# brson/synth2

Hardware: AMD Instinct MI355X
Metric: voice-samples/sec (mono) at 64k voices per GPU, 48 kHz, 1024-frame buffers (higher is better)
Workload: dtype f32

## Files before the change

### synth2_amd/csrc/s2r_aux.hip

```cpp
#include "s2r_kern_common.h"

namespace {

__global__ void __launch_bounds__(256) s2r_table_kernel(const S2rTabBuild b) {
    __shared__ uint64_t sT[S2R_EXP2F_N];
    if (threadIdx.x < S2R_EXP2F_N) sT[threadIdx.x] = c_exp2f_table[threadIdx.x];
    __syncthreads();
    const uint32_t i = blockIdx.x * blockDim.x + threadIdx.x;
    if (i >= b.n_entries) return;
    const S2rEnv &e = b.mod;
    float mod;
    bool dead = false;
    if (i < b.n_ad) {
        const float t = (float)i;
        const EnvRun s = env_stage_at(e, __builtin_inff(), __builtin_inff(), t);
        mod = env_value(s, t);
    } else if (i < b.n_ad + b.n_rel) {
        const float t = (float)(b.rc_t0 + (i - b.n_ad));
        mod = e.slope_rel * (t - e.sus_off) + e.S;
    } else if (i < b.n_ad + 2u * b.n_rel) {
        const float d = (float)(i - b.n_ad - b.n_rel);
        mod = e.slope_rel * d + e.S;
    } else if (i < b.n_ad + 2u * b.n_rel + 16u) {
        mod = 0.0f * 1.0f + e.S;
    } else {
        mod = 0.0f;
        dead = i >= b.n_ad + 2u * b.n_rel + 32u;
    }
    const float f_lpf = s2r_pow2_sleef_core(mod * b.amt_lpf) * b.lpf_freq;
    float c0, c1, c2 = 0.0f;
    if (b.lpf_kind == S2R_FILT_ONEPOLE) {
        const float num = (-2.0f * 3.14159274101257324f) * f_lpf;
        const float arg = b.fast_div_sr ? s2r_div_const_nocheck(num, b.sr, b.rcp_sr) : (num / b.sr);
        c0 = s2r_expf(arg, sT);
        c1 = 1.0f - c0;
        if (dead) { c0 = 1.0f; c1 = 0.0f; }
    } else {
        const FiltCoef fc = dsp_filter_coef(b.lpf_kind, b.lpf_damping, b.sr, f_lpf);
        c0 = fc.alpha; c1 = fc.beta; c2 = fc.gamma;
        if (dead) c0 = 1.0f;
    }
    b.base[i] = c0;
    b.base[(size_t)b.plane + i] = c1;
    if (b.lpf_kind != S2R_FILT_ONEPOLE) b.base[2u * (size_t)b.plane + i] = c2;
    if (b.fm_plane) b.base[(size_t)b.fm_plane * b.plane + i] = dead ? 1.0f : s2r_pow2_sleef_core(mod * b.amt_osc);
}

__global__ void __launch_bounds__(256) s2r_noise_table_kernel(float *t) {
    const uint32_t x = blockIdx.x * blockDim.x + threadIdx.x;
    const float f = (float)((x * 0x79b9u) & 0xffffu) * 0x1p-16f;
    const float q = __builtin_fmaf(f, 0x1.0001p-16f, f);
    t[x] = __builtin_fmaf(q, 2.0f, -1.0f);
}

__device__ __forceinline__ void mix_body(const S2rMixParams &m, uint32_t block, float *s_run) {
    const bool ov = m.ov_render_counter != nullptr;
    if (ov) {
        if (threadIdx.x == 0 && !ov_wait(m.ov_render_counter, m.ov_render_target)) ov_raise(m.ov_fail, 2u);
        __syncthreads();
    }
    mix_block(m, block, s_run, ov, m.done.flag != nullptr);
    signal_done(m.done, (m.frames + 15u) / 16u);
}

__global__ void __launch_bounds__(256) s2r_mix_kernel(const S2rMixParams m) {
    extern __shared__ float s_run[];
    tl_mark(m.timeline, m.tl_slot, 0);
    mix_body(m, blockIdx.x, s_run);
    tl_mark(m.timeline, m.tl_slot, 1);
}

__global__ void s2r_sum_rows_kernel(const float *rows, uint32_t n_rows, uint32_t frames, uint32_t stride, int stereo, float *out, const S2rDone done) {
    const uint32_t f = blockIdx.x * blockDim.x + threadIdx.x;
    if (f < frames) {
        float total = 0.0f;
        for (uint32_t r = 0; r < n_rows; ++r) total += rows[(size_t)r * stride + f];
        if (stereo) { out_store(done, out + 2u * f, total); out_store(done, out + 2u * f + 1u, total); }
        else out_store(done, out + f, total);
    }
    signal_done(done, gridDim.x);
}

constexpr int kDecimTaps = 63;
__global__ void s2r_decimate4_kernel(const float *x, const float *h, uint32_t n_out, float *out) {
    const uint32_t n = blockIdx.x * blockDim.x + threadIdx.x;
    if (n >= n_out) return;
    float acc = 0.0f;
    for (int k = 0; k < kDecimTaps; ++k) acc = acc + h[k] * x[4u * n + (uint32_t)k];
    out[n] = acc;
}
__global__ void s2r_decimate4_history_kernel(float *x, uint32_t n_out) {
    const uint32_t i = threadIdx.x;
    float v = 0.0f;
    if (i < kDecimTaps - 1) v = x[4u * n_out + i];
    __syncthreads();
    if (i < kDecimTaps - 1) x[i] = v;
}

__device__ __forceinline__ void heads_body(int32_t *heads, const S2rTimedEvent *tev, S2rTimedEvent *tev_copy, uint32_t n, uint32_t i, bool ov) {
    if (i >= n) return;
    const S2rTimedEvent e = tev[i];
    if (ov) {
        static_assert(sizeof(S2rTimedEvent) == 32, "two 16-byte stores");
        float *dst = reinterpret_cast<float *>(tev_copy + i);
        ov_store4(dst, (f4){s2r_u2f(e.voice), s2r_u2f(e.frame), s2r_u2f(e.flags), e.pitch});
        ov_store4(dst + 4, (f4){s2r_u2f(e.seed), s2r_u2f((uint32_t)e.next), s2r_u2f(e.program), 0.0f});
        if (e.flags & S2R_TEV_FIRST) ov_store(heads + e.voice, (int32_t)i);
    } else {
        tev_copy[i] = e;
        if (e.flags & S2R_TEV_FIRST) heads[e.voice] = (int32_t)i;
    }
}

__global__ void s2r_tev_heads_kernel(int32_t *heads, const S2rTimedEvent *tev, S2rTimedEvent *tev_copy, uint32_t n, uint32_t *ov_heads_counter) {
    heads_body(heads, tev, tev_copy, n, blockIdx.x * blockDim.x + threadIdx.x, ov_heads_counter != nullptr);
    if (ov_heads_counter != nullptr) ov_signal(ov_heads_counter);
}

__global__ void __launch_bounds__(256) s2r_mix_and_heads_kernel(const S2rMixParams m, uint32_t mix_blocks, int32_t *heads,
                                                                const S2rTimedEvent *tev, S2rTimedEvent *tev_copy, uint32_t n) {
    extern __shared__ float s_run[];
    tl_mark(m.timeline, m.tl_slot, 0);
    if (blockIdx.x < mix_blocks) mix_body(m, blockIdx.x, s_run);
    else {
        heads_body(heads, tev, tev_copy, n, (blockIdx.x - mix_blocks) * blockDim.x + threadIdx.x, m.ov_heads_counter != nullptr);
        if (m.ov_heads_counter != nullptr) ov_signal(m.ov_heads_counter);
    }
    tl_mark(m.timeline, m.tl_slot, 1);
}

__global__ void s2r_events_kernel(const S2rVoiceArrays v, const S2rVoiceEvent *ev, uint32_t n) {
    const uint32_t i = blockIdx.x * blockDim.x + threadIdx.x;
    if (i >= n) return;
    const S2rVoiceEvent e = ev[i];
    const uint32_t vi = e.voice;
    if (e.flags & S2R_EV_RESTART) {
        v.pitch[vi] = e.pitch;
        v.offset[vi] = 0u;
        v.release[vi] = 0u;
        v.flags[vi] = S2R_VF_STARTED | ((e.flags & S2R_EV_RELEASE) ? S2R_VF_RELEASED : 0u);
        v.phase[vi] = 0.0f;
        v.lpf_last[vi] = 0.0f;
        v.fx1[vi] = 0.0f; v.fx2[vi] = 0.0f; v.fy1[vi] = 0.0f; v.fy2[vi] = 0.0f;
        v.seed[vi] = e.seed;
        v.program[vi] = e.flags >> S2R_EV_PROGRAM_SHIFT;
        v.osc_z[vi] = s2r_u2f(S2R_OSC_Z_NONE);
    } else if (e.flags & S2R_EV_RELEASE) {
        const uint32_t fl = v.flags[vi];
        if ((fl & S2R_VF_STARTED) && !(fl & S2R_VF_RELEASED)) {
            v.release[vi] = v.offset[vi];
            v.flags[vi] = fl | S2R_VF_RELEASED;
        }
    }
}
}

hipError_t s2r_launch_onepole_resident_osc0(const S2rRenderArgs &a, const S2rResident &rs, uint32_t block_voices, hipStream_t stream);
hipError_t s2r_launch_onepole_resident_osc1(const S2rRenderArgs &a, const S2rResident &rs, uint32_t block_voices, hipStream_t stream);
hipError_t s2r_launch_onepole_resident_osc2(const S2rRenderArgs &a, const S2rResident &rs, uint32_t block_voices, hipStream_t stream);
hipError_t s2r_launch_onepole_resident_osc3(const S2rRenderArgs &a, const S2rResident &rs, uint32_t block_voices, hipStream_t stream);
hipError_t s2r_launch_onepole_pool_osc0(const S2rRenderArgs &a, const S2rPool &pl, uint32_t block_voices, hipStream_t stream);
hipError_t s2r_launch_onepole_pool_osc1(const S2rRenderArgs &a, const S2rPool &pl, uint32_t block_voices, hipStream_t stream);
hipError_t s2r_launch_onepole_pool_osc2(const S2rRenderArgs &a, const S2rPool &pl, uint32_t block_voices, hipStream_t stream);
hipError_t s2r_launch_onepole_pool_osc3(const S2rRenderArgs &a, const S2rPool &pl, uint32_t block_voices, hipStream_t stream);
hipError_t s2r_launch_onepole_osc0(const S2rRenderArgs &a, uint32_t block_voices, hipStream_t stream);
hipError_t s2r_launch_onepole_osc1(const S2rRenderArgs &a, uint32_t block_voices, hipStream_t stream);
hipError_t s2r_launch_onepole_osc2(const S2rRenderArgs &a, uint32_t block_voices, hipStream_t stream);
hipError_t s2r_launch_onepole_osc3(const S2rRenderArgs &a, uint32_t block_voices, hipStream_t stream);
hipError_t s2r_launch_general_pool_osc0(const S2rRenderArgs &a, const S2rPool &pl, uint32_t block_voices, hipStream_t stream);
hipError_t s2r_launch_general_pool_osc1(const S2rRenderArgs &a, const S2rPool &pl, uint32_t block_voices, hipStream_t stream);
hipError_t s2r_launch_general_pool_osc2(const S2rRenderArgs &a, const S2rPool &pl, uint32_t block_voices, hipStream_t stream);
hipError_t s2r_launch_general_pool_osc3(const S2rRenderArgs &a, const S2rPool &pl, uint32_t block_voices, hipStream_t stream);
hipError_t s2r_launch_general_pool_osc15(const S2rRenderArgs &a, const S2rPool &pl, uint32_t block_voices, hipStream_t stream);
hipError_t s2r_launch_general_osc0(const S2rRenderArgs &a, uint32_t block_voices, hipStream_t stream);
hipError_t s2r_launch_general_osc1(const S2rRenderArgs &a, uint32_t block_voices, hipStream_t stream);
hipError_t s2r_launch_general_osc2(const S2rRenderArgs &a, uint32_t block_voices, hipStream_t stream);
hipError_t s2r_launch_general_osc3(const S2rRenderArgs &a, uint32_t block_voices, hipStream_t stream);
hipError_t s2r_launch_general_osc15(const S2rRenderArgs &a, uint32_t block_voices, hipStream_t stream);

hipError_t s2r_launch_tables(const S2rTabBuild &b, hipStream_t stream) {
    if (b.n_entries == 0) return hipErrorInvalidValue;
    hipLaunchKernelGGL(s2r_table_kernel, dim3((b.n_entries + 255u) / 256u), dim3(256), 0, stream, b);
    return hipGetLastError();
}

hipError_t s2r_launch_noise_table(float *table_65536, hipStream_t stream) {
    hipLaunchKernelGGL(s2r_noise_table_kernel, dim3(65536 / 256), dim3(256), 0, stream, table_65536);
    return hipGetLastError();
}

hipError_t s2r_launch_render(const S2rRenderArgs &a, uint32_t block_voices, hipStream_t stream) {
    const S2rRenderParams &p = a.p;
    if (p.n_voices == 0 || p.frames == 0) return hipSuccess;
    if (block_voices < 64 || block_voices > 1024 || (block_voices & 63u)) return hipErrorInvalidValue;
    if (p.bank_size > 1 || p.osc_kind > S2R_OSC_SINE) return s2r_launch_general_osc15(a, block_voices, stream);
    const bool general = p.lpf_kind != S2R_FILT_ONEPOLE;
    switch (p.osc_kind) {
    case S2R_OSC_SQUARE: return general ? s2r_launch_general_osc0(a, block_voices, stream) : s2r_launch_onepole_osc0(a, block_voices, stream);
    case S2R_OSC_SAW: return general ? s2r_launch_general_osc1(a, block_voices, stream) : s2r_launch_onepole_osc1(a, block_voices, stream);
    case S2R_OSC_TRIANGLE: return general ? s2r_launch_general_osc2(a, block_voices, stream) : s2r_launch_onepole_osc2(a, block_voices, stream);
    case S2R_OSC_SINE: return general ? s2r_launch_general_osc3(a, block_voices, stream) : s2r_launch_onepole_osc3(a, block_voices, stream);
    default: return hipErrorInvalidValue;
    }
}

hipError_t s2r_launch_resident(const S2rRenderArgs &a, const S2rResident &rs, uint32_t block_voices, hipStream_t stream) {
    const S2rRenderParams &p = a.p;
    if (p.n_voices == 0 || p.frames == 0 || p.bank_size > 1 || p.lpf_kind != S2R_FILT_ONEPOLE) return hipErrorInvalidValue;
    switch (p.osc_kind) {
    case S2R_OSC_SQUARE: return s2r_launch_onepole_resident_osc0(a, rs, block_voices, stream);
    case S2R_OSC_SAW: return s2r_launch_onepole_resident_osc1(a, rs, block_voices, stream);
    case S2R_OSC_TRIANGLE: return s2r_launch_onepole_resident_osc2(a, rs, block_voices, stream);
    case S2R_OSC_SINE: return s2r_launch_onepole_resident_osc3(a, rs, block_voices, stream);
    default: return hipErrorInvalidValue;
    }
}

hipError_t s2r_launch_pool(const S2rRenderArgs &a, const S2rPool &pl, uint32_t block_voices, hipStream_t stream) {
    const S2rRenderParams &p = a.p;
    if (p.n_voices == 0 || p.frames == 0) return hipErrorInvalidValue;
    if (p.bank_size > 1 || p.osc_kind > S2R_OSC_SINE) return s2r_launch_general_pool_osc15(a, pl, block_voices, stream);
    const bool general = p.lpf_kind != S2R_FILT_ONEPOLE;
    switch (p.osc_kind) {
    case S2R_OSC_SQUARE: return general ? s2r_launch_general_pool_osc0(a, pl, block_voices, stream) : s2r_launch_onepole_pool_osc0(a, pl, block_voices, stream);
    case S2R_OSC_SAW: return general ? s2r_launch_general_pool_osc1(a, pl, block_voices, stream) : s2r_launch_onepole_pool_osc1(a, pl, block_voices, stream);
    case S2R_OSC_TRIANGLE: return general ? s2r_launch_general_pool_osc2(a, pl, block_voices, stream) : s2r_launch_onepole_pool_osc2(a, pl, block_voices, stream);
    case S2R_OSC_SINE: return general ? s2r_launch_general_pool_osc3(a, pl, block_voices, stream) : s2r_launch_onepole_pool_osc3(a, pl, block_voices, stream);
    default: return hipErrorInvalidValue;
    }
}

hipError_t s2r_launch_mix(const S2rMixParams &m, hipStream_t stream) {
    if (m.frames == 0) return hipSuccess;
    const uint32_t runs_per_group = (m.blocks_per_group + kMixRun - 1) / kMixRun;
    const size_t lds = (size_t)runs_per_group * m.n_groups * 16u * sizeof(float);
    if (lds > 64u * 1024u) return hipErrorInvalidValue;
    hipLaunchKernelGGL(s2r_mix_kernel, dim3((m.frames + 15) / 16), dim3(256), lds, stream, m);
    return hipGetLastError();
}

hipError_t s2r_launch_mix_and_heads(const S2rMixParams &m, int32_t *heads, const S2rTimedEvent *tev, S2rTimedEvent *tev_copy, uint32_t n,
                                    hipStream_t stream) {
    if (m.frames == 0) return s2r_launch_tev_heads(heads, tev, tev_copy, n, stream, m.ov_heads_counter);
    if (n == 0) return s2r_launch_mix(m, stream);
    const uint32_t runs_per_group = (m.blocks_per_group + kMixRun - 1) / kMixRun;
    const size_t lds = (size_t)runs_per_group * m.n_groups * 16u * sizeof(float);
    if (lds > 64u * 1024u) return hipErrorInvalidValue;
    const uint32_t mix_blocks = (m.frames + 15) / 16;
    hipLaunchKernelGGL(s2r_mix_and_heads_kernel, dim3(mix_blocks + (n + 255) / 256), dim3(256), lds, stream, m, mix_blocks, heads, tev, tev_copy, n);
    return hipGetLastError();
}

hipError_t s2r_launch_events(const S2rVoiceArrays &v, const S2rVoiceEvent *dev_events, uint32_t n, hipStream_t stream) {
    if (n == 0) return hipSuccess;
    hipLaunchKernelGGL(s2r_events_kernel, dim3((n + 255) / 256), dim3(256), 0, stream, v, dev_events, n);
    return hipGetLastError();
}

hipError_t s2r_launch_tev_heads(int32_t *heads, const S2rTimedEvent *tev, S2rTimedEvent *tev_copy, uint32_t n, hipStream_t stream,
                                uint32_t *ov_heads_counter) {
    if (n == 0) return hipSuccess;
    hipLaunchKernelGGL(s2r_tev_heads_kernel, dim3((n + 255) / 256), dim3(256), 0, stream, heads, tev, tev_copy, n, ov_heads_counter);
    return hipGetLastError();
}

hipError_t s2r_launch_decimate4(float *x_with_history, const float *taps, uint32_t n_out, float *out, hipStream_t stream) {
    if (n_out == 0) return hipSuccess;
    hipLaunchKernelGGL(s2r_decimate4_kernel, dim3((n_out + 255) / 256), dim3(256), 0, stream, x_with_history, taps, n_out, out);
// ... 12 lines not shown
```

### synth2_amd/csrc/s2r_device.h

```cpp
#pragma once
#include <hip/hip_runtime_api.h>
#include <stdint.h>
#include "s2r.h"

#define S2R_VF_STARTED 1u
#define S2R_VF_RELEASED 2u

struct S2rEnv {
    float A;
    float D;
    float S;
    float R;
    float sus_off;
    float slope_att;
    float slope_dec;
    float slope_rel;
};

struct S2rVoiceArrays {
    float *pitch;
    uint32_t *offset;
    uint32_t *release;
    uint32_t *flags;
    float *phase;
// ... 8 lines not shown

struct S2rBankEntry {
    int32_t osc_kind;
    float osc_gain, noise_level, lpf_freq, amt_osc, amt_lpf;
    int32_t lpf_kind;
    float lpf_shape;
    S2rEnv amp, mod;
    uint32_t tab_valid;
    uint32_t tab_off, tab_plane;
    int32_t tab_ad, tab_rc;
    uint32_t tab_rc_t0;
    int32_t tab_ru, tab_sus, tab_end, tab_dead;
};

struct S2rTimedEvent;

struct S2rDone {
    uint32_t *flag;
    uint32_t value;
    uint32_t *counter;
};

struct S2rTabRef {
    const float *base;
    uint32_t plane;
    int32_t ad;
    int32_t rc;
    uint32_t rc_t0;
    int32_t ru;
    int32_t sus;
    int32_t end;
    int32_t dead;
    uint32_t fm_plane;
};
#define S2R_TAB_PAD 16u
#define S2R_TAB_MAX_ENTRIES (1u << 22)

struct S2rMixTail {
    uint32_t n_mixers;
    uint32_t n_blocks, blocks_per_group, n_groups;
    int32_t root_add, stereo;
    float *out;
    S2rDone done;
    uint32_t *rows_done;
    uint32_t rows_target;
    int32_t xmode;
    uint32_t n_rows, row_stride;
    const float *rows;
    float *final_out;
    S2rDone final_done;
    int32_t final_stereo;
    unsigned long long *granules;
    uint32_t granule_tag;
};

struct S2rRenderParams {
    int32_t osc_kind;
    float osc_gain;
    float noise_level;
    float lpf_freq;
    float amt_osc;
    float amt_lpf;
    int32_t lpf_kind;
    float lpf_damping;
    S2rEnv amp;
    S2rEnv mod;
    float sr;
    float rcp_sr;
    int32_t fast_div_sr;
    int32_t no_flat_shortcut;
    uint32_t frames;
    uint32_t n_voices;
    uint32_t frames_stride;
    uint32_t super_frames;
    S2rVoiceArrays v;
    float *block_partials;
    float *direct_out;
    int32_t direct_stereo;
    S2rDone done;
    float *per_voice;
    const float *sin_table;
    const float *noise_tab;
    S2rTabRef tab;
    const S2rTimedEvent *tev;
    int32_t *voice_ev_head;
    unsigned long long *stamps;
    unsigned long long *timeline;
    uint32_t tl_slot;
    const S2rBankEntry *bank;
    uint32_t bank_size;
    const uint32_t *ov_heads_counter;
    uint32_t ov_heads_target;
    uint32_t *ov_render_counter;
    uint32_t *ov_fail;
    const S2rTimedEvent *tev_src;
    S2rTimedEvent *tev_copy;
    const uint32_t *slices;
    uint32_t *arrive;
    uint32_t arrive_target;
    S2rMixTail mt;
};

struct S2rVoiceEvent {
    uint32_t voice;
    uint32_t flags;
    float pitch;
    uint32_t seed;
};
#define S2R_EV_RESTART 1u
#define S2R_EV_RELEASE 2u
#define S2R_EV_PROGRAM_SHIFT 16

struct S2rTimedEvent {
    uint32_t voice;
    uint32_t frame;
    uint32_t flags;
    float pitch;
    uint32_t seed;
    int32_t next;
    uint32_t program;
    uint32_t _pad;
};
#define S2R_TEV_FIRST 0x100u

#define S2R_ARG_MAX_EVENTS 288u
struct S2rRenderArgs {
    S2rRenderParams p;
    uint32_t n_events;
    uint32_t _pad;
    uint32_t ev[3 * S2R_ARG_MAX_EVENTS];
};
static_assert(sizeof(S2rRenderArgs) <= 4096, "kernel arguments are limited to 4 KiB");

#define S2R_RES_CMD_WORDS 32u
#define S2R_RES_MAX_EVENTS 9u
#define S2R_RES_FLAG_EXIT 1u
#define S2R_RES_GRANULE_FRAMES 64u
struct S2rResident {
    const uint32_t *cmd;
    uint32_t *exited;
    uint32_t launch_id;
    uint32_t first_seq;
    uint32_t idle_ticks;
    uint32_t max_polls;
    uint32_t *done_flag, *done_counter;
    unsigned long long *granules;
};

#define S2R_POOL_CMD_SLOTS 4u
#define S2R_POOL_CMD_WORDS 16u
#define S2R_POOL_FLAG_EXIT 1u
#define S2R_POOL_FLAG_TWO_STREAMS 2u
struct S2rPool {
    const uint32_t *cmd;
    const uint32_t *slices;
    uint32_t slices_stride;
    const S2rTimedEvent *tev_src[4];
    S2rTimedEvent *tev_copy[2];
    int32_t *heads[2];
    float *partials[2];
    uint32_t *arrive;
    const uint32_t *ov_heads;
    uint32_t *ov_render;
    float *out[3];
    uint32_t *done_flag, *done_counter;
    uint32_t *decided;
    uint32_t *exited;
    uint32_t *fail;
    uint32_t launch_id, first_seq, idle_ticks, max_polls;
    S2rMixTail mt;
    float *rows[2], *rows_mine[2];
    float *final_out[3];
    uint32_t *final_flag, *final_counter;
    unsigned long long *granules;
};

struct S2rTabBuild {
    S2rEnv mod;
    float lpf_freq, amt_lpf, amt_osc, sr, rcp_sr;
    int32_t fast_div_sr;
    int32_t lpf_kind;
    float lpf_damping;
    float *base;
    uint32_t plane, n_ad, n_rel, n_entries;
    uint32_t rc_t0;
    uint32_t fm_plane;
};

struct S2rOverlapWords { uint32_t render_done[2], heads_done[2]; };

struct S2rMixParams {
    const float *block_partials;
    uint32_t n_blocks;
    uint32_t blocks_per_group;
    uint32_t n_groups;
    uint32_t frames;
    uint32_t frames_stride;
    int32_t root_add;
    int32_t stereo;
    float *out;
    S2rDone done;
    const uint32_t *ov_render_counter;
    uint32_t ov_render_target;
    uint32_t *ov_heads_counter;
    uint32_t *ov_fail;
    unsigned long long *timeline;
    uint32_t tl_slot;
    unsigned long long *granules;
    uint32_t granule_tag;
};

hipError_t s2r_launch_tables(const S2rTabBuild &b, hipStream_t stream);
hipError_t s2r_launch_noise_table(float *table_65536, hipStream_t stream);
hipError_t s2r_launch_resident(const S2rRenderArgs &a, const S2rResident &rs, uint32_t block_voices, hipStream_t stream);
hipError_t s2r_launch_render(const S2rRenderArgs &a, uint32_t block_voices, hipStream_t stream);
hipError_t s2r_launch_pool(const S2rRenderArgs &a, const S2rPool &pl, uint32_t block_voices, hipStream_t stream);
hipError_t s2r_launch_mix(const S2rMixParams &p, hipStream_t stream);
hipError_t s2r_launch_events(const S2rVoiceArrays &v, const S2rVoiceEvent *dev_events, uint32_t n, hipStream_t stream);
hipError_t s2r_launch_mix_and_heads(const S2rMixParams &m, int32_t *heads, const S2rTimedEvent *tev, S2rTimedEvent *tev_copy, uint32_t n,
                                    hipStream_t stream);
hipError_t s2r_launch_tev_heads(int32_t *heads, const S2rTimedEvent *tev, S2rTimedEvent *tev_copy, uint32_t n, hipStream_t stream,
                                uint32_t *ov_heads_counter = nullptr);
hipError_t s2r_launch_decimate4(float *x_with_history, const float *taps, uint32_t n_out, float *out, hipStream_t stream);
hipError_t s2r_launch_sum_rows(const float *rows, uint32_t n_rows, uint32_t frames, uint32_t stride, int stereo, float *out, hipStream_t stream,
                               const S2rDone *done);
```

### synth2_amd/csrc/s2r_host.cpp

```cpp
#include <hip/hip_runtime.h>
#include <cmath>
#include <cstdarg>
#include <cstdio>
#include <cstdlib>
#include <cstring>
#include <ctime>
#include <atomic>
#include <memory>
#include <new>
#include <string>
#include <vector>

#include "s2r.h"
#include "s2r_device.h"
#include "s2r_math.h"
#include "s2r_patch.h"
#include "s2r_voices.h"

namespace {

constexpr int kEventSlots = 4;
constexpr size_t kVoiceWords = S2R_VOICE_WORDS;

constexpr uint32_t kSinTableCrc = 0x55293b66u;
// ... 92 lines not shown
    int device = 0;
    uint32_t shard_begin = 0, shard_voices = 0, padded_voices = 0, block_voices = 256, n_blocks = 0, mix_groups = 1;
    uint32_t interleave = 0, shard_index = 0, shard_count = 1;
    FastDiv div_interleave, div_count, div_per_kid;
    std::vector<s2r_patch> bank;
    uint32_t program = 0;
    S2rBankEntry *bank_dev = nullptr;
    bool bank_dirty = true; uint32_t bank_rate = 0;
    std::shared_ptr<S2rVoicePool> pool;
    s2r_synth *parent = nullptr;
    std::vector<s2r_synth *> kids;
    float *rows_dev[2] = {nullptr, nullptr};
    std::vector<float *> kid_stage;
    std::vector<hipEvent_t> kid_done[2];
    uint32_t rows_slot = 0;
    std::vector<uint32_t> seed_override;
    std::vector<S2rVoiceEvent> pending;
    std::vector<int32_t> pending_slot;
    EventSlot slots[kEventSlots];
    int next_slot = 0;
    std::vector<S2rTimedEvent> tpending;
    std::vector<int32_t> tlast;
    std::vector<int32_t> tfirst;
    uint32_t fill_time = 0;
    uint32_t tev_capacity = 0;
    int32_t *voice_ev_head = nullptr;
    S2rTimedEvent *tev_copy = nullptr;
    hipStream_t stream = nullptr;
    S2rVoiceArrays v{};
    void *voice_mem = nullptr;
    float *block_partials = nullptr;
    float *out_dev = nullptr;
    float *out_host = nullptr;
    float *out_host_dev = nullptr;
    uint32_t *done_host = nullptr, *done_dev = nullptr, *done_counter = nullptr;
    uint32_t done_seq = 0;
    uint32_t ring_seq[2] = {0, 0};
    float *ring_host[2] = {nullptr, nullptr}, *ring_dev[2] = {nullptr, nullptr};
    hipEvent_t ring_done[2] = {nullptr, nullptr};
    size_t ring_frames[2] = {0, 0};
    uint32_t ring_head = 0, ring_count = 0;
    struct DeferredMix { bool active = false; bool overlap = false; S2rMixParams m{}; int ring_slot = -1; } dmix;
    hipStream_t stream_b = nullptr;
    bool ov_enabled = false;
    bool ov_registered = false;
    bool ov_busy = false;
    float *partials2[2] = {nullptr, nullptr};
    int32_t *heads2[2] = {nullptr, nullptr};
    S2rTimedEvent *tevcopy2[2] = {nullptr, nullptr};
    S2rOverlapWords *ov_words = nullptr;
    uint32_t ov_render_target[2] = {0, 0}, ov_heads_target[2] = {0, 0};
    uint32_t ov_fill = 0;
    int fused_mode = 1;
    uint32_t *fz_arrive = nullptr;
    uint32_t fz_target[2] = {0, 0};
    FastDiv div_block;
    std::vector<S2rTimedEvent> tsorted;
    std::vector<uint32_t> tperm, tbounds;
    uint32_t *rows_done = nullptr;
    uint32_t rows_target[2] = {0, 0};
    bool xg_on = false;
    uint32_t xg_rank = 0, xg_n = 0, xg_target[2] = {0, 0};
    float *xg_rows = nullptr;
    uint32_t *xg_done = nullptr;
    void *xg_block = nullptr; bool xg_owner = false;
    bool force_stage = false, force_peer = false;
    bool resident = false, pool_running = false;
    uint32_t pool_seq = 0, pool_launch_id = 0, pool_rate = 0, pool_fills = 0;
    uint32_t *pool_cmd = nullptr, *pool_cmd_dev = nullptr; bool pool_cmd_vram = false;
    uint32_t *pool_slices = nullptr, *pool_slices_dev = nullptr;
    uint32_t *pool_host = nullptr, *pool_host_dev = nullptr;
    uint32_t *pool_decided = nullptr;
    bool pool_gran_pending = false;
    EventSlot *pool_gran_slot = nullptr;
    volatile uint32_t *pool_staged = nullptr; uint32_t pool_staged_seq = 0;
    uint32_t pool_idle_ticks = 200000u;
    int n_cu = 0;
    float *os_buf = nullptr, *os_taps = nullptr;
    float *sin_dev = nullptr;
    float *noise_dev = nullptr;
    float *per_voice_dev = nullptr; size_t per_voice_cap = 0;
    float *tab_dev = nullptr; size_t tab_cap = 0;
    S2rTabRef tab{};
    bool tab_dirty = true; uint32_t tab_rate = 0;
    float *bank_tab_dev = nullptr; size_t bank_tab_cap = 0;
    unsigned long long *stamps_dev = nullptr;
    unsigned long long *timeline_dev = nullptr; uint32_t timeline_n = 0, timeline_cap = 0;
    bool use_tab = true, use_arg_events = true;
    bool low_latency = false, res_running = false, res_stereo = false;
    uint32_t res_rate = 0, res_seq = 0, res_launch_id = 0;
    uint32_t *res_host = nullptr, *res_dev = nullptr;
    unsigned long long *res_gran = nullptr, *res_gran_dev = nullptr;
    uint32_t *res_cmd = nullptr;
    uint32_t *res_cmd_dev = nullptr;
    bool res_cmd_vram = false;
    float pitch_table[256];
    hipEvent_t t0 = nullptr, t1 = nullptr;
    bool timing = false, timed = false, no_flat_shortcut = false;
    uint64_t double_release = 0;
    s2r_voice_log_fn voice_log = nullptr;
    void *voice_log_user = nullptr;
    bool broken = false;
    std::string err = "";
};


namespace {

int set_err(s2r_synth *s, int code, const char *fmt, ...) {
    if (s) {
        char buf[512];
        va_list ap; va_start(ap, fmt); vsnprintf(buf, sizeof buf, fmt, ap); va_end(ap);
        s->err = buf;
    }
    return code;
}

#define S2R_QUIESCE(s) do { const int rc_q_ = quiesce(s); if (rc_q_ != S2R_OK) return rc_q_; } while (0)
int resident_stop(s2r_synth *s);
int pool_stop(s2r_synth *s);
int quiesce(s2r_synth *s) { int rc = resident_stop(s); return rc != S2R_OK ? rc : pool_stop(s); }

#define S2R_HIP(s, call)                                                                              \
    do {                                                                                              \
        hipError_t e_ = (call);                                                                       \
        if (e_ != hipSuccess) return set_err((s), S2R_ERR_HIP, "%s failed: %s", #call, hipGetErrorString(e_)); \
    } while (0)

inline int64_t to_local(const s2r_synth *s, uint32_t pool_index) {
    if (s->interleave == 0) {
        if (pool_index < s->shard_begin || pool_index >= s->shard_begin + s->shard_voices) return -1;
        return (int64_t)(pool_index - s->shard_begin);
    }
    const uint32_t run = s->div_interleave.div(pool_index), within = pool_index - run * s->interleave;
    const uint32_t lrun = s->div_count.div(run);
    if (run - lrun * s->shard_count != s->shard_index) return -1;
    return (int64_t)(lrun * s->interleave + within);
}
inline uint32_t to_pool(const s2r_synth *s, uint32_t local) {
    if (s->interleave == 0) return s->shard_begin + local;
    const uint32_t lrun = s->div_interleave.div(local);
    return (lrun * s->shard_count + s->shard_index) * s->interleave + (local - lrun * s->interleave);
}

inline s2r_synth *shard_of(s2r_synth *s, uint32_t pool_index, uint32_t *local) {
    if (!s->kids.empty()) {
        const uint32_t k = s->interleave ? s->div_count.mod(s->div_interleave.div(pool_index)) : s->div_per_kid.div(pool_index);
        s = s->kids[k];
    }
    const int64_t mine = to_local(s, pool_index);
    if (mine < 0) return nullptr;
    *local = (uint32_t)mine;
    return s;
}

void push_event(s2r_synth *top, uint32_t pool_index, uint32_t flags, float pitch, uint32_t seed, uint32_t program = 0) {
    uint32_t local = 0;
    s2r_synth *s = shard_of(top, pool_index, &local);
    if (!s) return;
    int32_t slot = s->pending_slot[local];
    if (slot < 0) {
        slot = (int32_t)s->pending.size();
        s->pending_slot[local] = slot;
        s->pending.push_back(S2rVoiceEvent{local, 0u, 0.0f, 0u});
    }
    S2rVoiceEvent &e = s->pending[(size_t)slot];
// ... 130 lines not shown
                s->dmix.active = false;
                S2rMixParams m = s->dmix.m;
                m.ov_heads_counter = hc;
                if (s2r_launch_mix_and_heads(m, s->heads2[ov_parity], sl.tdev, s->tevcopy2[ov_parity], nt, s->stream_b) != hipSuccess) {
                    s->ov_heads_target[ov_parity] -= (nt + 255u) / 256u; s->broken = true;
                    return set_err(s, S2R_ERR_HIP, "the launch of the chain heads and the mix failed");
                }
            } else {
                if (s2r_launch_tev_heads(s->heads2[ov_parity], sl.tdev, s->tevcopy2[ov_parity], nt, s->stream_b, hc) != hipSuccess) {
                    s->ov_heads_target[ov_parity] -= (nt + 255u) / 256u; s->broken = true;
                    return set_err(s, S2R_ERR_HIP, "the launch of the chain heads failed");
                }
            }
            *timed_slot = &sl; *tev_dev = s->tevcopy2[ov_parity];
        } else if (s->dmix.active && stream == s->stream) {
            s->dmix.active = false;
            S2R_HIP(s, s2r_launch_mix_and_heads(s->dmix.m, s->voice_ev_head, sl.tdev, s->tev_copy, nt, stream));
            *timed_slot = &sl; *tev_dev = s->tev_copy;
        } else {
            S2R_HIP(s, s2r_launch_tev_heads(s->voice_ev_head, sl.tdev, s->tev_copy, nt, stream));
            *timed_slot = &sl; *tev_dev = s->tev_copy;
        }
        for (const S2rTimedEvent &e : s->tpending) s->tlast[e.voice] = -1;
        s->tpending.clear();
    } else if (done) {
        sl.state = 2; sl.word = s->done_host + (done->flag - s->done_dev); sl.seq = done->value;
    } else {
        S2R_HIP(s, hipEventRecord(sl.done, stream));
        sl.state = 1;
    }
    for (const S2rVoiceEvent &e : s->pending) s->pending_slot[e.voice] = -1;
    s->pending.clear();
    return S2R_OK;
}

#define S2R_REFUSE_BROKEN(s) do { if ((s)->broken) return set_err((s), S2R_ERR_HIP, "an earlier fill failed on the device (a bounded wait between kernels ran out): the device's voices no longer match the host's bookkeeping; destroy the handle"); } while (0)

int check_fill(s2r_synth *s, size_t frames, uint32_t sample_rate) {
    if (!s) return S2R_ERR_INVALID;
    S2R_REFUSE_BROKEN(s);
    if (frames > s->cfg.max_frames) return set_err(s, S2R_ERR_TOO_MANY_FRAMES, "frames %zu > max_frames %u", frames, s->cfg.max_frames);
    if (sample_rate == 0) return set_err(s, S2R_ERR_INVALID, "sample_rate_hz must be > 0");
    if (s->fill_time && s->fill_time >= frames)
        return set_err(s, S2R_ERR_INVALID, "a timed event at frame %u does not fall inside this %zu-frame fill", s->fill_time, frames);
    if (s->pool->oldest_offset() + (frames - s->fill_time) > 0xffffffffull)
        return set_err(s, S2R_ERR_OFFSET_OVERFLOW, "a voice's frame offset would overflow u32 (the reference panics here)");
    for (size_t k = 0; k < s->bank.size(); k++) {
        const s2r_patch &pt = s->bank[k];
        if (pt.lpf_kind == S2R_FILT_ONEPOLE) continue;
        const double amt = pt.mod_env_to_lpf_freq > 0.0f ? (double)pt.mod_env_to_lpf_freq : 0.0;
        const double num_max = 2.0 * 3.14159265358979323846 * (double)pt.lpf_freq * std::exp2(amt) * 1.000001;
        if (!(num_max < 3.4028234e38))
            return set_err(s, S2R_ERR_PATCH_RANGE, "patch %zu, lpf.kind %d: 2 pi * lpf.freq * 2^mod_env_to_lpf_freq overflows f32",
                           k, pt.lpf_kind);
        if (pt.lpf_kind == S2R_FILT_BP2 &&
            !(pt.lpf_q > 0.0f && num_max / (double)sample_rate / (2.0 * (double)pt.lpf_q) < 3.4028234e38))
            return set_err(s, S2R_ERR_PATCH_RANGE, "patch %zu: lpf.kind bp2 needs lpf.q > 0 (tan(theta / (2 q)) must stay finite)", k);
        if (pt.lpf_kind >= S2R_FILT_SVF_LP && !(pt.lpf_q >= 0x1p-100f))
            return set_err(s, S2R_ERR_PATCH_RANGE, "patch %zu: the state-variable filter needs lpf.q > 0 (k = 1 / q)", k);
    }
    return S2R_OK;
}

bool tables_wanted(const s2r_synth *s) {
    return s->use_tab && !s->no_flat_shortcut && s->bank.size() == 1 && s->bank[0].osc_kind <= S2R_OSC_SINE &&
           (s->bank[0].lpf_kind == S2R_FILT_ONEPOLE || s->block_voices <= 256u);
}

bool plan_tables(const S2rEnv &e, S2rTabBuild &b) {
    if (!(e.sus_off >= 0.0f && e.sus_off < (float)S2R_TAB_MAX_ENTRIES && e.R >= 0.0f && e.R < (float)S2R_TAB_MAX_ENTRIES)) return false;
    b.mod = e;
    b.rc_t0 = (uint32_t)std::ceil((double)e.sus_off);
    b.n_ad = b.rc_t0 + 1u + S2R_TAB_PAD;
    b.n_rel = (uint32_t)std::ceil((double)e.R) + 2u + S2R_TAB_PAD;
    b.n_entries = b.n_ad + 2u * b.n_rel + 48u;
    b.plane = (b.n_entries + 3u) & ~3u;
    return true;
}

int ensure_tables(s2r_synth *s, const S2rRenderParams &p, uint32_t sample_rate, hipStream_t stream) {
    if (!tables_wanted(s)) { return S2R_OK; }
    if (!s->tab_dirty && s->tab_rate == sample_rate) return S2R_OK;
    s->tab = S2rTabRef{};
    s->tab_dirty = false; s->tab_rate = sample_rate;
    S2rTabBuild b{};
    if (!plan_tables(p.mod, b)) return S2R_OK;
    b.lpf_freq = p.lpf_freq; b.amt_lpf = p.amt_lpf; b.amt_osc = p.amt_osc; b.sr = p.sr; b.rcp_sr = p.rcp_sr;
    b.fast_div_sr = p.fast_div_sr; b.lpf_kind = p.lpf_kind; b.lpf_damping = p.lpf_damping;
    const bool onepole = p.lpf_kind == S2R_FILT_ONEPOLE;
    const uint32_t n_planes = (onepole ? 2u : 3u) + (p.amt_osc != 0.0f ? 1u : 0u);
    b.fm_plane = p.amt_osc != 0.0f ? (onepole ? 2u : 3u) : 0u;
    const size_t need = (size_t)b.plane * n_planes;
    if (need > s->tab_cap) {
        S2R_HIP(s, hipStreamSynchronize(stream));
        S2R_HIP(s, hipStreamSynchronize(s->stream));
        if (s->tab_dev) { S2R_HIP(s, hipFree(s->tab_dev)); s->tab_dev = nullptr; s->tab_cap = 0; }
        S2R_HIP(s, hipMalloc((void **)&s->tab_dev, need * sizeof(float)));
        s->tab_cap = need;
    }
    b.base = s->tab_dev;
    S2R_HIP(s, s2r_launch_tables(b, stream));
    S2rTabRef &t = s->tab;
    t.base = s->tab_dev; t.plane = b.plane;
    t.ad = 0; t.rc = (int32_t)b.n_ad; t.rc_t0 = b.rc_t0; t.ru = (int32_t)(b.n_ad + b.n_rel);
    t.sus = (int32_t)(b.n_ad + 2u * b.n_rel); t.end = t.sus + 16; t.dead = t.sus + 32;
    t.fm_plane = b.fm_plane;
    return S2R_OK;
}

S2rRenderParams make_params(s2r_synth *s, size_t frames, uint32_t sample_rate) {
    S2rRenderParams p{};
    p.osc_kind = s->bank[0].osc_kind;
    p.osc_gain = s->bank[0].osc_gain;
    p.noise_level = s->bank[0].noise;
    p.lpf_freq = s->bank[0].lpf_freq;
    p.amt_osc = s->bank[0].mod_env_to_osc_freq;
    p.amt_lpf = s->bank[0].mod_env_to_lpf_freq;
    p.lpf_kind = s->bank[0].lpf_kind;
    p.lpf_damping = s->bank[0].lpf_kind >= S2R_FILT_BP2 ? s->bank[0].lpf_q : s->bank[0].lpf_damping;
    p.amp = resolve_env(s->bank[0].amp_env, sample_rate);
    p.mod = resolve_env(s->bank[0].mod_env, sample_rate);
    p.sr = (float)sample_rate;
    p.rcp_sr = 1.0f / p.sr;
    p.fast_div_sr = (fast_div_rate(sample_rate) && s->bank[0].lpf_freq >= 0x1p-30f && s->bank[0].lpf_freq <= 0x1p30f) ? 1 : 0;
    p.no_flat_shortcut = s->no_flat_shortcut ? 1 : 0;
    p.frames = (uint32_t)frames;
    p.n_voices = s->shard_voices;
    p.frames_stride = partials_stride(s->cfg.max_frames);
    p.v = s->v;
    p.block_partials = s->block_partials;
    p.per_voice = nullptr;
    p.sin_table = s->sin_dev;
    { static const bool off = [] { const char *e = std::getenv("S2R_NOISE_TAB"); return e && e[0] == '0'; }();
      p.noise_tab = off ? nullptr : s->noise_dev; }
    p.bank = s->bank_dev;
    p.bank_size = (uint32_t)s->bank.size();
    return p;
}

int ensure_bank(s2r_synth *s, uint32_t sample_rate, hipStream_t stream, bool *bank_kernel_out) {
    bool bank_kernel = s->bank.size() > 1;
    for (const s2r_patch &pt : s->bank) if (pt.osc_kind > S2R_OSC_SINE) bank_kernel = true;
    if (bank_kernel && (s->bank_dirty || s->bank_rate != sample_rate)) {
        std::vector<S2rBankEntry> host(s->bank.size());
        std::vector<S2rTabBuild> builds(s->bank.size());
        size_t tab_floats = 0;
        const float srf = (float)sample_rate;
        for (size_t k = 0; k < s->bank.size(); k++) {
            const s2r_patch &pt = s->bank[k];
            S2rBankEntry &e = host[k];
            std::memset(&e, 0, sizeof e);
            e.osc_kind = pt.osc_kind; e.osc_gain = pt.osc_gain; e.noise_level = pt.noise; e.lpf_freq = pt.lpf_freq;
            e.amt_osc = pt.mod_env_to_osc_freq; e.amt_lpf = pt.mod_env_to_lpf_freq; e.lpf_kind = pt.lpf_kind;
            e.lpf_shape = pt.lpf_kind >= S2R_FILT_BP2 ? pt.lpf_q : pt.lpf_damping;
            e.amp = resolve_env(pt.amp_env, sample_rate);
            e.mod = resolve_env(pt.mod_env, sample_rate);
            S2rTabBuild &b = builds[k];
            b = S2rTabBuild{};
            if (s->use_tab && !s->no_flat_shortcut && plan_tables(e.mod, b) && tab_floats + (size_t)b.plane * 4u <= ((size_t)1 << 28)) {
                b.lpf_freq = e.lpf_freq; b.amt_lpf = e.amt_lpf; b.amt_osc = e.amt_osc; b.sr = srf; b.rcp_sr = 1.0f / srf;
                b.fast_div_sr = 0;
                b.lpf_kind = e.lpf_kind; b.lpf_damping = e.lpf_shape; b.fm_plane = 3u;
                e.tab_valid = 1u; e.tab_off = (uint32_t)tab_floats; e.tab_plane = b.plane;
                e.tab_ad = 0; e.tab_rc = (int32_t)b.n_ad; e.tab_rc_t0 = b.rc_t0; e.tab_ru = (int32_t)(b.n_ad + b.n_rel);
                e.tab_sus = (int32_t)(b.n_ad + 2u * b.n_rel); e.tab_end = e.tab_sus + 16; e.tab_dead = e.tab_sus + 32;
                tab_floats += (size_t)b.plane * 4u;
            }
        }
        if (tab_floats > s->bank_tab_cap) {
            S2R_HIP(s, hipStreamSynchronize(stream));
            S2R_HIP(s, hipStreamSynchronize(s->stream));
            if (s->bank_tab_dev) { S2R_HIP(s, hipFree(s->bank_tab_dev)); s->bank_tab_dev = nullptr; s->bank_tab_cap = 0; }
            S2R_HIP(s, hipMalloc((void **)&s->bank_tab_dev, tab_floats * sizeof(float)));
            s->bank_tab_cap = tab_floats;
        }
        for (size_t k = 0; k < s->bank.size(); k++)
            if (host[k].tab_valid) { builds[k].base = s->bank_tab_dev + host[k].tab_off; S2R_HIP(s, s2r_launch_tables(builds[k], stream)); }
        S2R_HIP(s, hipMemcpyAsync(s->bank_dev, host.data(), host.size() * sizeof(S2rBankEntry), hipMemcpyHostToDevice, stream));
        S2R_HIP(s, hipStreamSynchronize(stream));
        s->bank_dirty = false; s->bank_rate = sample_rate;
    }
    *bank_kernel_out = bank_kernel;
    return S2R_OK;
}


struct Exchange {
    uint32_t *rows_done = nullptr;
    uint32_t rows_target = 0;
// ... 46 lines not shown
    s->tevcopy2[0] = s->tev_copy;
    if (s->tevcopy2[1]) {
        S2R_HIP(s, hipFree(s->tevcopy2[1])); s->tevcopy2[1] = nullptr;
        S2R_HIP(s, hipMalloc((void **)&s->tevcopy2[1], (size_t)cap * sizeof(S2rTimedEvent)));
    }
    s->tev_capacity = cap;
    return S2R_OK;
}

int fused_events(s2r_synth *s, hipStream_t stream, EventSlot **slot_out, uint32_t *nt_out) {
    *slot_out = nullptr; *nt_out = 0;
    merge_pending_into_chains(s);
    const uint32_t nt = (uint32_t)s->tpending.size();
    s->tbounds.assign((size_t)s->n_blocks + 1u, 0u);
    if (nt == 0) return S2R_OK;
    { int rc = ensure_tev_capacity(s, nt, stream); if (rc != S2R_OK) return rc; }
    EventSlot &sl = s->slots[s->next_slot];
    s->next_slot = (s->next_slot + 1) % kEventSlots;
    { int rc = slot_release(s, sl); if (rc != S2R_OK) return rc; }
    uint32_t *b = s->tbounds.data();
    for (const S2rTimedEvent &e : s->tpending) b[s->div_block.div(e.voice) + 1u]++;
    for (uint32_t k = 0; k < s->n_blocks; k++) b[k + 1u] += b[k];
    s->tperm.resize(nt);
    {
        static thread_local std::vector<uint32_t> cur;
        cur.assign(b, b + s->n_blocks);
        for (uint32_t i = 0; i < nt; i++) s->tperm[i] = cur[s->div_block.div(s->tpending[i].voice)]++;
    }
    s->tsorted.resize(nt);
    for (uint32_t i = 0; i < nt; i++) {
        S2rTimedEvent e = s->tpending[i];
        if (e.next >= 0) e.next = (int32_t)s->tperm[(size_t)e.next];
        s->tsorted[s->tperm[i]] = e;
    }
    std::memcpy(sl.thost, s->tsorted.data(), (size_t)nt * sizeof(S2rTimedEvent));
    for (const S2rTimedEvent &e : s->tpending) s->tlast[e.voice] = -1;
    s->tpending.clear();
    *slot_out = &sl; *nt_out = nt;
    return S2R_OK;
}

uint32_t pick_mixers(const s2r_synth *s, size_t frames) {
    uint32_t m = (uint32_t)((frames + 15u) / 16u);
    const uint32_t half = s->n_blocks > 1u ? s->n_blocks / 2u : 1u;
    if (m > half) m = half;
    if (m > 64u) m = 64u;
    return m ? m : 1u;
}

S2rMixTail mix_tail_of(const s2r_synth *s, bool root_add) {
    S2rMixTail mt{};
    mt.n_blocks = s->n_blocks;
    mt.n_groups = root_add ? s->mix_groups : 1u;
    mt.blocks_per_group = (s->n_blocks + mt.n_groups - 1u) / mt.n_groups;
    mt.root_add = root_add ? 1 : 0;
    return mt;
}

bool fused_shape_ok(const s2r_synth *s) {
    if (!s->fused_mode || s->n_blocks < 2u) return false;
    if (!onepole_single_patch(s) && s->block_voices > 256u) return false;
    if ((size_t)s->n_blocks + 1u > 3u * S2R_ARG_MAX_EVENTS) return false;
    const uint32_t groups = s->mix_groups ? s->mix_groups : 1u;
    const uint32_t runs = ((s->n_blocks + groups - 1u) / groups + 15u) / 16u * groups;
    return runs * 16u <= 16u * 32u;
}

int enqueue_fused(s2r_synth *s, size_t frames, uint32_t sample_rate, hipStream_t stream, float *dev_out, bool root_add, bool stereo,
                  const S2rDone *done, const Exchange *xc) {
    { int rc = overlap_drain(s); if (rc != S2R_OK) return rc; }
    { int rc = launch_deferred_mix(s, s->stream); if (rc != S2R_OK) return rc; }
    bool arg_events = s->use_arg_events && s->tpending.empty() && s->pending.size() <= S2R_ARG_MAX_EVENTS;
    if (arg_events)
        for (const S2rVoiceEvent &e : s->pending) if (e.seed != 0u) { arg_events = false; break; }
    EventSlot *slot = nullptr;
    uint32_t nt = 0;
    if (!arg_events) { int rc = fused_events(s, stream, &slot, &nt); if (rc != S2R_OK) return rc; }
    static thread_local S2rRenderArgs a;
    S2rRenderParams &p = a.p;
    bool bank_kernel = false;
    { int rc = ensure_bank(s, sample_rate, stream, &bank_kernel); if (rc != S2R_OK) return rc; }
    p = make_params(s, frames, sample_rate);
    { int rc = ensure_tables(s, p, sample_rate, stream); if (rc != S2R_OK) return rc; }
    if (tables_wanted(s)) p.tab = s->tab;
    else if (bank_kernel) { p.tab = S2rTabRef{}; p.tab.base = s->bank_tab_dev; }
    p.stamps = s->stamps_dev;
    if (s->timeline_dev && s->timeline_n < s->timeline_cap) { p.timeline = s->timeline_dev; p.tl_slot = s->timeline_n++; }
    p.voice_ev_head = s->voice_ev_head;
    p.ov_fail = s->done_dev + 3;
    a.n_events = 0;
    if (arg_events) {
        a.n_events = (uint32_t)s->pending.size();
        for (uint32_t i = 0; i < a.n_events; i++) {
            const S2rVoiceEvent &e = s->pending[i];
            a.ev[3u * i] = e.voice; a.ev[3u * i + 1u] = e.flags; a.ev[3u * i + 2u] = s2r_f2u(e.pitch);
        }
        for (const S2rVoiceEvent &e : s->pending) s->pending_slot[e.voice] = -1;
        s->pending.clear();
    } else if (slot) {
        p.tev = s->tev_copy; p.tev_copy = s->tev_copy; p.tev_src = slot->tdev; p.slices = nullptr;
        std::memcpy(a.ev, s->tbounds.data(), ((size_t)s->n_blocks + 1u) * sizeof(uint32_t));
    }
    p.arrive = s->fz_arrive;
    s->fz_target[0] += s->n_blocks;
    p.arrive_target = s->fz_target[0];
    S2rMixTail &mt = p.mt;
    mt = mix_tail_of(s, root_add);
    mt.n_mixers = pick_mixers(s, frames);
    mt.stereo = stereo ? 1 : 0;
    mt.out = dev_out;
    mt.done = done ? *done : S2rDone{nullptr, 0u, s->done_counter + 3};
    if (xc) {
        if (xc->xmode != 2) mt.done.flag = nullptr;
        mt.xmode = xc->xmode;
        mt.rows_done = xc->rows_done; mt.rows_target = xc->rows_target;
        mt.n_rows = xc->n_rows; mt.row_stride = xc->row_stride; mt.rows = xc->rows;
        mt.final_out = xc->final_out; mt.final_done = xc->final_done; mt.final_stereo = xc->final_stereo ? 1 : 0;
    }
    if (s->timing) S2R_HIP(s, hipEventRecord(s->t0, stream));
    S2R_HIP(s, s2r_launch_render(a, s->block_voices, stream));
    if (s->timing) { S2R_HIP(s, hipEventRecord(s->t1, stream)); s->timed = true; }
    if (slot) {
        if (xc && xc->slot_word) { slot->state = 2; slot->word = xc->slot_word; slot->seq = xc->final_done.value; }
        else if (done && done->flag) { slot->state = 2; slot->word = s->done_host + (done->flag - s->done_dev); slot->seq = done->value; }
        else { S2R_HIP(s, hipEventRecord(slot->done, stream)); slot->state = 1; }
    }
    if (!s->parent) {
        s->pool->advance(frames - s->fill_time);
        s->fill_time = 0;
    }
    return S2R_OK;
}


bool pool_exited(const s2r_synth *s) { return __atomic_load_n(&s->pool_host[0], __ATOMIC_ACQUIRE) == s->pool_launch_id; }

bool pool_eligible(const s2r_synth *s, size_t frames) {
    return s->resident && s->kids.empty() && s->pool_cmd != nullptr && fused_shape_ok(s) && (int)s->n_blocks <= s->n_cu && s->block_voices <= 256u &&
           !s->timing && s->timeline_dev == nullptr && frames <= 0xffffu && frames <= s->cfg.max_frames;
}

int pool_setup(s2r_synth *s) {
    if (s->pool_cmd) return S2R_OK;
    S2R_HIP(s, hipSetDevice(s->device));
    S2R_HIP(s, hipHostMalloc((void **)&s->pool_host, 16 * sizeof(uint32_t), kHostPolled));
    std::memset(s->pool_host, 0, 16 * sizeof(uint32_t));
    S2R_HIP(s, hipHostGetDevicePointer((void **)&s->pool_host_dev, s->pool_host, 0));
    const size_t sl_words = (size_t)S2R_POOL_CMD_SLOTS * (s->n_blocks + 1u);
    S2R_HIP(s, hipHostMalloc((void **)&s->pool_slices, sl_words * sizeof(uint32_t), kHostPolled));
    std::memset(s->pool_slices, 0, sl_words * sizeof(uint32_t));
    S2R_HIP(s, hipHostGetDevicePointer((void **)&s->pool_slices_dev, s->pool_slices, 0));
    S2R_HIP(s, hipMalloc((void **)&s->pool_decided, sizeof(uint32_t)));
    const size_t pv = s->padded_voices;
    if (!s->partials2[1]) S2R_HIP(s, hipMalloc((void **)&s->partials2[1], (size_t)s->n_blocks * partials_stride(s->cfg.max_frames) * sizeof(float)));
    if (!s->heads2[1]) {
        S2R_HIP(s, hipMalloc((void **)&s->heads2[1], pv * sizeof(int32_t)));
        S2R_HIP(s, hipMemset(s->heads2[1], 0xff, pv * sizeof(int32_t)));
    }
    if (!s->tevcopy2[1]) S2R_HIP(s, hipMalloc((void **)&s->tevcopy2[1], (size_t)s->tev_capacity * sizeof(S2rTimedEvent)));
    if (!s->res_gran) {
        S2R_HIP(s, hipHostMalloc((void **)&s->res_gran, S2R_RES_GRANULE_FRAMES * sizeof(unsigned long long), kHostPolled));
        std::memset(s->res_gran, 0, S2R_RES_GRANULE_FRAMES * sizeof(unsigned long long));
        S2R_HIP(s, hipHostGetDevicePointer((void **)&s->res_gran_dev, s->res_gran, 0));
    }
    const size_t cmd_words = (size_t)S2R_POOL_CMD_SLOTS * S2R_POOL_CMD_WORDS;
    int large_bar = 0;
    const char *force_host = std::getenv("S2R_RES_CMD_HOST");
    if (!(force_host && force_host[0] == '1') &&
        hipDeviceGetAttribute(&large_bar, hipDeviceAttributeIsLargeBar, s->device) == hipSuccess && large_bar) {
        uint32_t *v = nullptr;
        if (hipExtMallocWithFlags((void **)&v, cmd_words * sizeof(uint32_t), hipDeviceMallocFinegrained) == hipSuccess && v) {
            S2R_HIP(s, hipMemset(v, 0, cmd_words * sizeof(uint32_t)));
            S2R_HIP(s, hipDeviceSynchronize());
            s->pool_cmd = v; s->pool_cmd_dev = v; s->pool_cmd_vram = true;
        } else (void)hipGetLastError();
    }
    if (!s->pool_cmd) {
        uint32_t *h = nullptr;
        S2R_HIP(s, hipHostMalloc((void **)&h, cmd_words * sizeof(uint32_t), kHostPolled));
        std::memset(h, 0, cmd_words * sizeof(uint32_t));
        S2R_HIP(s, hipHostGetDevicePointer((void **)&s->pool_cmd_dev, h, 0));
        s->pool_cmd = h; s->pool_cmd_vram = false;
    }
    return S2R_OK;
}

hipError_t malloc_exchange(void **p, size_t bytes) {
    if (hipExtMallocWithFlags(p, bytes, hipDeviceMallocFinegrained) == hipSuccess && *p) return hipSuccess;
    (void)hipGetLastError();
    return hipMalloc(p, bytes);
}

volatile uint32_t *pool_post_payload(s2r_synth *s, const uint32_t *w, uint32_t *seq_out) {
    const uint32_t seq = ++s->pool_seq;
    volatile uint32_t *c = s->pool_cmd + (size_t)(seq % S2R_POOL_CMD_SLOTS) * S2R_POOL_CMD_WORDS;
    for (uint32_t i = 1; i < 15; i++) c[i] = w[i];
    *seq_out = seq;
    return c;
}
uint32_t pool_post(s2r_synth *s, const uint32_t *w) {
    uint32_t seq = 0;
    volatile uint32_t *c = pool_post_payload(s, w, &seq);
    if (s->pool_cmd_vram) store_fence();
    __atomic_store_n(&c[15], seq, __ATOMIC_RELEASE);
    if (s->pool_cmd_vram) store_fence();
    __atomic_store_n(&c[0], seq, __ATOMIC_RELEASE);
    if (s->pool_cmd_vram) store_fence();
    return seq;
}

int pool_stop(s2r_synth *s) {
    if (!s) return S2R_OK;
    for (s2r_synth *kid : s->kids) { int rc = pool_stop(kid); if (rc != S2R_OK) { s->err = kid->err; return rc; } }
    if (!s->pool_running) return S2R_OK;
    uint32_t w[16] = {0};
    w[1] = S2R_POOL_FLAG_EXIT << 16;
    (void)pool_post(s, w);
    s->pool_running = false;
    S2R_HIP(s, hipSetDevice(s->device));
    S2R_HIP(s, hipStreamSynchronize(s->stream));
    return S2R_OK;
}

int pool_launch(s2r_synth *s, uint32_t sample_rate, uint32_t first_seq) {
    S2R_HIP(s, hipSetDevice(s->device));
    static thread_local S2rRenderArgs a;
    S2rRenderParams &p = a.p;
    bool bank_kernel = false;
    { int rc = ensure_bank(s, sample_rate, s->stream, &bank_kernel); if (rc != S2R_OK) return rc; }
    p = make_params(s, s->cfg.max_frames, sample_rate);
    { int rc = ensure_tables(s, p, sample_rate, s->stream); if (rc != S2R_OK) return rc; }
    if (tables_wanted(s)) p.tab = s->tab;
    else if (bank_kernel) { p.tab = S2rTabRef{}; p.tab.base = s->bank_tab_dev; }
    p.voice_ev_head = s->voice_ev_head;
    p.stamps = s->stamps_dev;
    p.tev = s->tev_copy;
    a.n_events = 0;
    S2rPool pl{};
    pl.cmd = s->pool_cmd_dev; pl.slices = s->pool_slices_dev; pl.slices_stride = s->n_blocks + 1u;
    for (int k = 0; k < 4; k++) pl.tev_src[k] = s->slots[k].tdev;
    for (int b = 0; b < 2; b++) { pl.tev_copy[b] = s->tevcopy2[b]; pl.heads[b] = s->heads2[b]; pl.partials[b] = s->partials2[b]; }
    pl.arrive = s->fz_arrive;
    if (s->ov_words) { pl.ov_heads = s->ov_words->heads_done; pl.ov_render = s->ov_words->render_done; }
    pl.out[0] = s->ring_dev[0]; pl.out[1] = s->ring_dev[1]; pl.out[2] = s->out_host_dev;
    pl.done_flag = s->done_dev; pl.done_counter = s->done_counter;
    pl.decided = s->pool_decided; pl.exited = s->pool_host_dev; pl.fail = s->done_dev + 3;
    pl.granules = s->res_gran_dev;
    pl.launch_id = ++s->pool_launch_id; pl.first_seq = first_seq;
    pl.idle_ticks = s->pool_idle_ticks; pl.max_polls = 1u << 24;
    s2r_synth *par = s->parent;
    pl.mt = mix_tail_of(s, par == nullptr);
    if (par) {
        uint32_t k = 0;
        while (k < par->kids.size() && par->kids[k] != s) k++;
        pl.mt.rows_done = par->rows_done;
        pl.mt.n_rows = (uint32_t)par->kids.size(); pl.mt.row_stride = par->cfg.max_frames;
        for (int b = 0; b < 2; b++) { pl.rows[b] = par->rows_dev[b]; pl.rows_mine[b] = par->rows_dev[b] + (size_t)k * par->cfg.max_frames; }
        pl.final_out[0] = par->ring_dev[0]; pl.final_out[1] = par->ring_dev[1]; pl.final_out[2] = par->out_host_dev;
        pl.final_flag = par->done_dev; pl.final_counter = nullptr;
    }
    if (s->xg_on) {
        pl.mt = mix_tail_of(s, false);
        pl.mt.xmode = s->xg_rank == 0 ? 1 : 2;
        pl.mt.rows_done = s->xg_done; pl.mt.n_rows = s->xg_n; pl.mt.row_stride = s->cfg.max_frames;
        for (int b = 0; b < 2; b++) { pl.rows[b] = s->xg_rows + (size_t)b * s->xg_n * s->cfg.max_frames; pl.rows_mine[b] = pl.rows[b] + (size_t)s->xg_rank * s->cfg.max_frames; }
        pl.final_out[0] = s->ring_dev[0]; pl.final_out[1] = s->ring_dev[1]; pl.final_out[2] = s->out_host_dev;
        pl.final_flag = s->done_dev; pl.final_counter = nullptr;
    }
    S2R_HIP(s, hipMemsetD32Async((hipDeviceptr_t)s->pool_decided, (int)((first_seq - 1u) << 1), 1, s->stream));
    S2R_HIP(s, s2r_launch_pool(a, pl, s->block_voices, s->stream));
    s->pool_running = true; s->pool_rate = sample_rate;
    return S2R_OK;
}

int pool_recover(s2r_synth *s) {
    if (!s->pool_running || !pool_exited(s)) return S2R_OK;
    s->pool_running = false;
    const bool dbg = std::getenv("S2R_DEBUG_STUCK") != nullptr;
    if (dbg) std::fprintf(stderr, "[s2r rank %u] pool_recover: kernel %u has left; pool_seq %u\n", s->xg_rank, s->pool_launch_id, s->pool_seq);
    S2R_HIP(s, hipSetDevice(s->device));
    S2R_HIP(s, hipStreamSynchronize(s->stream));
    uint32_t d = 0;
    S2R_HIP(s, hipMemcpy(&d, s->pool_decided, sizeof d, hipMemcpyDeviceToHost));
    const uint32_t first = (d & 1u) ? (d >> 1) : (d >> 1) + 1u;
    if (dbg) std::fprintf(stderr, "[s2r rank %u] pool_recover: decided %u -> first pending %u\n", s->xg_rank, d, first);
    if ((int32_t)(s->pool_seq - first) < 0) return S2R_OK;
    const int rc = pool_launch(s, s->pool_rate, first);
    if (dbg) std::fprintf(stderr, "[s2r rank %u] pool_recover: launched again (%d)\n", s->xg_rank, rc);
    return rc;
}

int pool_fill(s2r_synth *s, size_t frames, uint32_t sample_rate, uint32_t sel, bool stereo, uint32_t done_value, const Exchange *xc, uint32_t rows_slot,
              bool stage_only = false) {
    { int rc = overlap_drain(s); if (rc != S2R_OK) return rc; }
    { int rc = launch_deferred_mix(s, s->stream); if (rc != S2R_OK) return rc; }
    if (s->pool_running && (s->pool_rate != sample_rate || pool_exited(s) || s->pending.size() + s->tpending.size() > s->tev_capacity)) {
        int rc = pool_exited(s) ? pool_recover(s) : S2R_OK;
        if (rc == S2R_OK) rc = pool_stop(s);
        if (rc != S2R_OK) return rc;
    }
    EventSlot *slot = nullptr;
    uint32_t nt = 0;
    { int rc = fused_events(s, s->stream, &slot, &nt); if (rc != S2R_OK) return rc; }
    const uint32_t par = s->pool_fills++ & 1u;
    s->fz_target[par] += s->n_blocks;
    uint32_t w[16] = {0};
    w[1] = (uint32_t)frames; w[2] = nt; w[3] = done_value; w[4] = sel | (stereo ? 256u : 0u);
    w[5] = slot ? (uint32_t)(slot - s->slots) : 0u; w[6] = par; w[7] = s->fz_target[par]; w[8] = pick_mixers(s, frames);
    w[9] = xc ? xc->rows_target : 0u; w[10] = rows_slot;
    s->pool_gran_pending = sel == 2u && !xc && frames <= S2R_RES_GRANULE_FRAMES && s->res_gran != nullptr;
    w[12] = s->pool_gran_pending ? 1u : 0u;
    const uint32_t next_seq = s->pool_seq + 1u;
    std::memcpy(s->pool_slices + (size_t)(next_seq % S2R_POOL_CMD_SLOTS) * (s->n_blocks + 1u), s->tbounds.data(), ((size_t)s->n_blocks + 1u) * sizeof(uint32_t));
    std::atomic_thread_fence(std::memory_order_release);
    uint32_t seq = 0;
    if (stage_only && s->pool_running) { s->pool_staged = pool_post_payload(s, w, &seq); s->pool_staged_seq = seq; }
    else seq = pool_post(s, w);
    if (!s->pool_running) { int rc = pool_launch(s, sample_rate, seq); if (rc != S2R_OK) return rc; }
    s->pool_gran_slot = nullptr;
    if (slot) {
        slot->state = 2; slot->seq = done_value;
        slot->word = (xc && xc->slot_word) ? xc->slot_word : s->done_host + sel;
        if (s->pool_gran_pending) s->pool_gran_slot = slot;
    }
    if (!s->parent) {
        s->pool->advance(frames - s->fill_time);
        s->fill_time = 0;
    }
    return S2R_OK;
}

int enqueue_fill(s2r_synth *s, size_t frames, uint32_t sample_rate, hipStream_t stream, float *dev_out,
                 bool root_add, bool stereo, float *per_voice_dev, int defer_ring_slot = -1, const S2rDone *done = nullptr,
                 const Exchange *xc = nullptr, bool via_pool = false) {
    if (dev_out != nullptr && per_voice_dev == nullptr && fused_shape_ok(s) &&
        (xc != nullptr || s->fused_mode >= 2 || !(s->ov_enabled && defer_ring_slot >= 0 && stream == s->stream && root_add && done != nullptr)))
        return enqueue_fused(s, frames, sample_rate, stream, dev_out, root_add, stereo, done, xc);
    if (s->dmix.active && stream != s->stream) {
        int rc = launch_deferred_mix(s, s->stream);
        if (rc != S2R_OK) return rc;
        S2R_HIP(s, hipStreamSynchronize(s->stream));
    }
    const bool overlap = s->ov_enabled && defer_ring_slot >= 0 && stream == s->stream && dev_out != nullptr && root_add && s->n_blocks > 1 &&
                         per_voice_dev == nullptr && done != nullptr;
    const int ov_parity = overlap ? (int)(s->ov_fill & 1u) : -1;
    if (!overlap) { int rc = overlap_drain(s); if (rc != S2R_OK) return rc; }
    else if (s->dmix.active && !s->dmix.overlap) { int rc = launch_deferred_mix(s, stream); if (rc != S2R_OK) return rc; }
    bool arg_events = s->use_arg_events && s->tpending.empty() && s->pending.size() <= S2R_ARG_MAX_EVENTS;
    if (arg_events)
        for (const S2rVoiceEvent &e : s->pending) if (e.seed != 0u) { arg_events = false; break; }
    via_pool = via_pool && overlap;
    if (via_pool) {
        if (s->pool_running && (s->pool_rate != sample_rate || pool_exited(s) || s->pending.size() + s->tpending.size() > s->tev_capacity)) {
            int rc = pool_exited(s) ? pool_recover(s) : S2R_OK;
            if (rc == S2R_OK) rc = pool_stop(s);
            if (rc != S2R_OK) return rc;
        }
        arg_events = false;
        merge_pending_into_chains(s);
    }
    EventSlot *timed_slot = nullptr;
    const S2rTimedEvent *tev_dev = nullptr;
    if (!arg_events) {
        int rc = flush_events(s, stream, &timed_slot, &tev_dev, done, ov_parity);
        if (rc != S2R_OK) return rc;
    }
    {
        int rc = launch_deferred_mix(s, stream);
        if (rc != S2R_OK) return rc;
    }
    bool bank_kernel = false;
    { int rc = ensure_bank(s, sample_rate, stream, &bank_kernel); if (rc != S2R_OK) return rc; }
    static thread_local S2rRenderArgs a;
    S2rRenderParams &p = a.p;
    p = make_params(s, frames, sample_rate);
    {
        int rc = ensure_tables(s, p, sample_rate, stream);
        if (rc != S2R_OK) return rc;
    }
    if (tables_wanted(s)) p.tab = s->tab;
    else if (bank_kernel) { p.tab = S2rTabRef{}; p.tab.base = s->bank_tab_dev; }
    p.stamps = s->stamps_dev;
    if (s->timeline_dev && s->timeline_n < s->timeline_cap) { p.timeline = s->timeline_dev; p.tl_slot = s->timeline_n++; }
    p.per_voice = per_voice_dev;
    p.tev = tev_dev;
    p.voice_ev_head = s->voice_ev_head;
    if (overlap) {
        p.block_partials = s->partials2[ov_parity];
        p.voice_ev_head = s->heads2[ov_parity];
        if (tev_dev) { p.ov_heads_counter = &s->ov_words->heads_done[ov_parity]; p.ov_heads_target = s->ov_heads_target[ov_parity]; }
        p.ov_render_counter = &s->ov_words->render_done[ov_parity];
        p.ov_fail = s->done_dev + 3;
        s->ov_render_target[ov_parity] += s->n_blocks;
    }
    a.n_events = 0;
    if (arg_events) {
        a.n_events = (uint32_t)s->pending.size();
        for (uint32_t i = 0; i < a.n_events; i++) {
            const S2rVoiceEvent &e = s->pending[i];
            a.ev[3u * i] = e.voice; a.ev[3u * i + 1u] = e.flags; a.ev[3u * i + 2u] = s2r_f2u(e.pitch);
        }
        for (const S2rVoiceEvent &e : s->pending) s->pending_slot[e.voice] = -1;
        s->pending.clear();
    }
    const bool direct = dev_out != nullptr && root_add && s->n_blocks == 1;
    if (direct) { p.direct_out = dev_out; p.direct_stereo = stereo ? 1 : 0; if (done) p.done = *done; }
    if (via_pool) {
        uint32_t w[16] = {0};
        w[1] = (uint32_t)frames | (S2R_POOL_FLAG_TWO_STREAMS << 16); w[2] = tev_dev ? 1u : 0u; w[6] = (uint32_t)ov_parity;
        w[11] = s->ov_heads_target[ov_parity];
        const uint32_t seq = pool_post(s, w);
        if (!s->pool_running) { int rc = pool_launch(s, sample_rate, seq); if (rc != S2R_OK) return rc; }
    } else {
    if (s->timing) S2R_HIP(s, hipEventRecord(s->t0, stream));
    if (s2r_launch_render(a, s->block_voices, stream) != hipSuccess) {
        if (overlap) { s->ov_render_target[ov_parity] -= s->n_blocks; s->broken = true; }
        return set_err(s, S2R_ERR_HIP, "the render kernel's launch failed: %s", hipGetErrorString(hipGetLastError()));
    }
    if (s->timing) { S2R_HIP(s, hipEventRecord(s->t1, stream)); s->timed = true; }
    }
    if (timed_slot) {
        if (done) { timed_slot->state = 2; timed_slot->word = s->done_host + (done->flag - s->done_dev); timed_slot->seq = done->value; }
        else { S2R_HIP(s, hipEventRecord(timed_slot->done, stream)); timed_slot->state = 1; }
    }
    if (dev_out && !direct) {
        S2rMixParams m{};
        m.block_partials = s->block_partials;
        m.n_blocks = s->n_blocks;
        m.n_groups = root_add ? s->mix_groups : 1u;
        m.blocks_per_group = (s->n_blocks + m.n_groups - 1) / m.n_groups;
        m.frames = (uint32_t)frames;
        m.frames_stride = partials_stride(s->cfg.max_frames);
        m.root_add = root_add ? 1 : 0;
        m.stereo = stereo ? 1 : 0;
        m.out = dev_out;
        if (done) m.done = *done;
        if (s->timeline_dev && s->timeline_n < s->timeline_cap) { m.timeline = s->timeline_dev; m.tl_slot = s->timeline_n++; }
        if (overlap) {
            m.block_partials = s->partials2[ov_parity];
            m.ov_render_counter = &s->ov_words->render_done[ov_parity];
            m.ov_render_target = s->ov_render_target[ov_parity];
            m.ov_fail = s->done_dev + 3;
            s->ov_fill++;
            s->ov_busy = true;
        }
        if (defer_ring_slot >= 0 && stream == s->stream) { s->dmix.active = true; s->dmix.overlap = overlap; s->dmix.m = m; s->dmix.ring_slot = defer_ring_slot; }
        else S2R_HIP(s, s2r_launch_mix(m, stream));
    }
    if (!s->parent) {
        s->pool->advance(frames - s->fill_time);
        s->fill_time = 0;
    }
    return S2R_OK;
}


int enqueue_multi(s2r_synth *s, size_t frames, uint32_t sample_rate, float *dev_out, bool stereo, float *per_voice_host = nullptr,
                  const S2rDone *done = nullptr, int rows_slot_in = -1) {
    const uint32_t n = (uint32_t)s->kids.size();
    const uint32_t slot = rows_slot_in >= 0 ? (uint32_t)rows_slot_in : ((s->ring_head + s->ring_count) & 1u) ^ 1u;
    bool exchange = done != nullptr && done->flag != nullptr && !per_voice_host && s->rows_done != nullptr;
    for (uint32_t k = 0; k < n && exchange; k++) exchange = fused_shape_ok(s->kids[k]) && s->kid_stage[k] == nullptr;
    if (exchange) s->rows_target[slot] += n;
// ... 89 lines not shown
    S2R_HIP(s, hipStreamSynchronize(s->stream));
    if (s->stream_b) S2R_HIP(s, hipStreamSynchronize(s->stream_b));
    if ((int32_t)(*f - seq) < 0) return set_err(s, S2R_ERR_HIP, "the fill's last kernel finished without signalling completion");
    return S2R_OK;
}

int overlap_check(s2r_synth *s) {
    uint32_t who = *(volatile uint32_t *)(s->done_host + 3);
    s->done_host[3] = 0u;
    for (s2r_synth *kid : s->kids) { const uint32_t w = *(volatile uint32_t *)(kid->done_host + 3); kid->done_host[3] = 0u; if (w) who = w; }
    if (who == 0u) return S2R_OK;
    s->broken = true;
    return set_err(s, S2R_ERR_HIP, "%s gave up waiting for another kernel's or workgroup's work: the fill's output is not valid",
                   who == 1u ? "a render kernel (for its chain heads)" : who == 2u ? "a mix (for its partial rows)" : "the sum of the shards' rows (for a shard's row)");
}

int enqueue_root(s2r_synth *s, size_t frames, uint32_t sample_rate, float *dev_out, bool stereo, int defer_ring_slot = -1,
                 const S2rDone *done = nullptr) {
    if (!s->kids.empty()) return enqueue_multi(s, frames, sample_rate, dev_out, stereo, nullptr, done, defer_ring_slot);
    if (s->xg_on) {
        if (!(done && done->flag) || !fused_shape_ok(s))
            return set_err(s, S2R_ERR_INVALID, "a handle in a process group fills through s2r_fill / s2r_fill_begin, with more than one workgroup (of at most 256 voices unless the patch is a single one-pole one)");
        const uint32_t slot = defer_ring_slot >= 0 ? (uint32_t)defer_ring_slot : ((s->ring_head + s->ring_count) & 1u) ^ 1u;
        Exchange xc;
        s->xg_target[slot] += s->xg_n;
        xc.xmode = s->xg_rank == 0 ? 1 : 2;
        xc.rows_done = s->xg_done + slot; xc.rows_target = s->xg_target[slot];
        xc.n_rows = s->xg_n; xc.row_stride = s->cfg.max_frames; xc.rows = s->xg_rows + (size_t)slot * s->xg_n * s->cfg.max_frames;
        xc.final_out = dev_out; xc.final_done = *done; xc.final_stereo = stereo;
        xc.slot_word = s->done_host + (done->flag - s->done_dev);
        float *row = s->xg_rows + ((size_t)slot * s->xg_n + s->xg_rank) * s->cfg.max_frames;
        if (pool_eligible(s, frames)) return pool_fill(s, frames, sample_rate, (uint32_t)(done->flag - s->done_dev), stereo, done->value, &xc, slot);
        { int rc = pool_stop(s); if (rc != S2R_OK) return rc; }
        return enqueue_fill(s, frames, sample_rate, s->stream, row, false, false, nullptr, -1, done, &xc);
    }
    if (done && done->flag && pool_eligible(s, frames)) {
        static const bool fused_only = [] { const char *e = std::getenv("S2R_POOL_FORM"); return e && e[0] == 'f'; }();
        if (s->ov_enabled && defer_ring_slot >= 0 && !stereo && !fused_only)
            return enqueue_fill(s, frames, sample_rate, s->stream, dev_out, true, stereo, nullptr, defer_ring_slot, done, nullptr, true);
        return pool_fill(s, frames, sample_rate, (uint32_t)(done->flag - s->done_dev), stereo, done->value, nullptr, 0u);
    }
    { int rc = pool_stop(s); if (rc != S2R_OK) return rc; }
    return enqueue_fill(s, frames, sample_rate, s->stream, dev_out, true, stereo, nullptr, defer_ring_slot, done);
}


void resident_post(s2r_synth *s, uint32_t seq) {
    volatile uint32_t *c = s->res_cmd;
    if (s->res_cmd_vram) store_fence();
    __atomic_store_n(&c[31], seq, __ATOMIC_RELEASE);
    if (s->res_cmd_vram) store_fence();
    __atomic_store_n(&c[0], seq, __ATOMIC_RELEASE);
    if (s->res_cmd_vram) store_fence();
}

bool resident_exited(const s2r_synth *s) { return __atomic_load_n(&s->res_host[32], __ATOMIC_ACQUIRE) == s->res_launch_id; }

int resident_stop(s2r_synth *s) {
    if (!s || !s->res_running) return S2R_OK;
    volatile uint32_t *c = s->res_cmd;
    c[1] = S2R_RES_FLAG_EXIT << 16; c[2] = 0; c[3] = 0;
    resident_post(s, ++s->res_seq);
    s->res_running = false;
    S2R_HIP(s, hipSetDevice(s->device));
    S2R_HIP(s, hipStreamSynchronize(s->stream));
    return S2R_OK;
}

bool resident_eligible(const s2r_synth *s, size_t frames) {
    if (!s->low_latency || s->parent || !s->kids.empty() || s->n_blocks != 1 || s->block_voices > 256u) return false;
    if (s->bank.size() != 1 || s->bank[0].osc_kind > S2R_OSC_SINE || s->bank[0].lpf_kind != S2R_FILT_ONEPOLE) return false;
    if (!s->use_arg_events || !s->tpending.empty() || s->fill_time != 0 || s->pending.size() > S2R_RES_MAX_EVENTS) return false;
    if (s->timing || s->dmix.active || s->ring_count != 0 || s->timeline_dev || frames > 0xffffu) return false;
    for (const S2rVoiceEvent &e : s->pending) if (e.seed != 0u) return false;
    return true;
}

int resident_launch(s2r_synth *s, uint32_t sample_rate, bool stereo) {
    S2R_HIP(s, hipSetDevice(s->device));
    static thread_local S2rRenderArgs a;
    S2rRenderParams &p = a.p;
    p = make_params(s, s->cfg.max_frames, sample_rate);
    { int rc = ensure_tables(s, p, sample_rate, s->stream); if (rc != S2R_OK) return rc; }
    if (tables_wanted(s)) p.tab = s->tab;
    p.voice_ev_head = s->voice_ev_head;
    p.direct_out = s->out_host_dev; p.direct_stereo = stereo ? 1 : 0;
    p.stamps = s->stamps_dev;
    a.n_events = 0;
    S2rResident rs{};
    rs.cmd = s->res_cmd_dev; rs.exited = s->res_dev + 32;
    rs.launch_id = ++s->res_launch_id;
    rs.first_seq = s->res_seq + 1u;
    rs.idle_ticks = 100000u;
    rs.max_polls = 1u << 20;
    rs.done_flag = s->done_dev + 2; rs.done_counter = s->done_counter + 2;
    rs.granules = s->res_gran_dev;
    S2R_HIP(s, s2r_launch_resident(a, rs, s->block_voices, s->stream));
    s->res_running = true; s->res_rate = sample_rate; s->res_stereo = stereo;
    return S2R_OK;
}

int resident_fill(s2r_synth *s, float *out, size_t frames, uint32_t sample_rate, bool stereo) {
    if (s->res_running && (s->res_rate != sample_rate || s->res_stereo != stereo || resident_exited(s))) {
        int rc = resident_stop(s);
        if (rc != S2R_OK) return rc;
    }
    if (!s->res_running) { int rc = resident_launch(s, sample_rate, stereo); if (rc != S2R_OK) return rc; }
    volatile uint32_t *c = s->res_cmd;
    const uint32_t n = (uint32_t)s->pending.size();
    const uint32_t done_value = ++s->done_seq;
    c[1] = (uint32_t)frames; c[2] = n; c[3] = done_value;
    for (uint32_t i = 0; i < n; i++) {
        const S2rVoiceEvent &e = s->pending[i];
        c[4u + 3u * i] = e.voice; c[5u + 3u * i] = e.flags; c[6u + 3u * i] = s2r_f2u(e.pitch);
    }
    for (const S2rVoiceEvent &e : s->pending) s->pending_slot[e.voice] = -1;
    s->pending.clear();
    resident_post(s, ++s->res_seq);
    s->pool->advance(frames);
    volatile uint32_t *f = s->done_host + 2;
    const bool gran = frames <= S2R_RES_GRANULE_FRAMES && s->res_gran != nullptr;
    volatile unsigned long long *g = s->res_gran;
    auto arrived = [&]() -> bool {
        if (!gran) return (int32_t)(*f - done_value) >= 0;
        for (size_t i = frames; i-- > 0;) if ((uint32_t)(g[i] >> 32) != done_value) return false;
        return true;
    };
    bool done = false;
    for (int attempt = 0; attempt < 3 && !done; attempt++) {
        for (int round = 0; round < 4000 && !done; round++) {
            for (int i = 0; i < 1000; i++) {
                if (arrived()) { done = true; break; }
                cpu_relax();
            }
            if (!done && resident_exited(s)) break;
        }
        if (done || arrived()) { done = true; break; }
        if (!resident_exited(s)) break;
        s->res_running = false;
        S2R_HIP(s, hipSetDevice(s->device));
        S2R_HIP(s, hipStreamSynchronize(s->stream));
        if (arrived()) { done = true; break; }
        int rc = resident_launch(s, sample_rate, stereo);
        if (rc != S2R_OK) return rc;
        resident_post(s, ++s->res_seq);
    }
    if (!done) {
        (void)resident_stop(s);
        if (!arrived()) return set_err(s, S2R_ERR_HIP, "the resident kernel did not report the fill");
    }
    if (gran) {
        for (size_t i = 0; i < frames; i++) {
            const float v = s2r_u2f((uint32_t)g[i]);
            if (stereo) { out[2 * i] = v; out[2 * i + 1] = v; } else out[i] = v;
        }
        return S2R_OK;
    }
    std::atomic_thread_fence(std::memory_order_acquire);
    std::memcpy(out, s->out_host, frames * (stereo ? 2 : 1) * sizeof(float));
    return S2R_OK;
}

int fill_host(s2r_synth *s, float *out, size_t frames, uint32_t sample_rate, bool stereo) {
    int rc = check_fill(s, frames, sample_rate);
    if (rc != S2R_OK) return rc;
    if (frames == 0) return S2R_OK;
    if (!out) return set_err(s, S2R_ERR_INVALID, "null output buffer");
// ... 1096 lines not shown
```

### synth2_amd/csrc/s2r_kern_common.h

```cpp
#pragma once
#include <hip/hip_runtime.h>
#include <type_traits>
#include "s2r_device.h"
#include "s2r_math.h"

namespace {

__constant__ uint64_t c_exp2f_table[S2R_EXP2F_N] = S2R_EXP2F_TABLE_INIT;

constexpr int kChunk = 16;
constexpr uint32_t kSuperMax = 256;
constexpr uint32_t kSuperWhole = 1024;
constexpr int kP = 4;
constexpr uint32_t kTileRow = 68;

typedef float f4 __attribute__((ext_vector_type(4)));
typedef int i4 __attribute__((ext_vector_type(4)));
typedef unsigned u4 __attribute__((ext_vector_type(4)));
typedef unsigned short us4 __attribute__((ext_vector_type(4)));
typedef double d4 __attribute__((ext_vector_type(4)));
typedef unsigned long long ul4 __attribute__((ext_vector_type(4)));

__device__ __forceinline__ f4 vfma(f4 a, f4 b, f4 c) { return __builtin_elementwise_fma(a, b, c); }
__device__ __forceinline__ d4 vfma(d4 a, d4 b, d4 c) { return __builtin_elementwise_fma(a, b, c); }
// ... 956 lines not shown
                    }
                }
                d = (uint32_t)__builtin_amdgcn_readlane((int)d, 0);
                if (d == bail_word) { leave = true; break; }
                decided_run = d == run_word || (int32_t)((d >> 1) - want) > 0;
                if (decided_run && complete) {
                    if (lane < S2R_POOL_CMD_WORDS) s_cmd[lane] = w;
                    const uint32_t n_rec = (uint32_t)__builtin_amdgcn_readlane((int)w, 2);
                    if (lane >= 16u && lane < 18u)
                        s_cmd[lane] = n_rec == 0u ? 0u : __hip_atomic_load(pl.slices + (size_t)slot * pl.slices_stride + blockIdx.x + (lane - 16u), __ATOMIC_RELAXED, __HIP_MEMORY_SCOPE_SYSTEM);
                    break;
                }
                ++polls;
                const bool out_of_patience = __builtin_amdgcn_s_memrealtime() - t0 > (unsigned long long)pl.idle_ticks || polls >= pl.max_polls;
                if (out_of_patience) {
                    if (decided_run) { leave = true; break; }
                    uint32_t won = 0u;
                    if (lane == 0u) {
                        uint32_t expected = last << 1;
                        won = __hip_atomic_compare_exchange_strong(pl.decided, &expected, bail_word, __ATOMIC_RELAXED, __ATOMIC_RELAXED, __HIP_MEMORY_SCOPE_AGENT) ? 1u : 0u;
                        if (!won && expected == bail_word) won = 1u;
                    }
                    if (__builtin_amdgcn_readlane((int)won, 0) != 0) { leave = true; break; }
                    decided_run = true;
                    polls = pl.max_polls > 4096u ? pl.max_polls - 4096u : 0u;
                }
                if (polls < 128u) __builtin_amdgcn_s_sleep(1); else __builtin_amdgcn_s_sleep(8);
            }
            if (leave && lane == 0u) s_cmd[1] = S2R_POOL_FLAG_EXIT << 16;
        }
        __syncthreads();
        const uint32_t w1 = s_cmd[1];
        if ((w1 >> 16) & S2R_POOL_FLAG_EXIT) break;
        last = s_cmd[0];
        const uint32_t frames = w1 & 0xffffu, sel = s_cmd[4] & 0xffu, par = s_cmd[6] & 1u, es = s_cmd[5] & 3u;
        const int32_t stereo = (int32_t)((s_cmd[4] >> 8) & 1u);
        FillCtl ctl = FillCtl{};
        ctl.frames = frames; ctl.n_events = 0u;
        ctl.partials = par ? pl.partials[1] : pl.partials[0];
        ctl.heads = par ? pl.heads[1] : pl.heads[0];
        ctl.tev_copy = par ? pl.tev_copy[1] : pl.tev_copy[0];
        ctl.tev = ctl.tev_copy;
        ctl.tev_src = es == 0u ? pl.tev_src[0] : es == 1u ? pl.tev_src[1] : es == 2u ? pl.tev_src[2] : pl.tev_src[3];
        ctl.slice_lo = s_cmd[16]; ctl.slice_hi = s_cmd[17];
        ctl.fail = pl.fail;
        const bool two_streams = ((w1 >> 16) & S2R_POOL_FLAG_TWO_STREAMS) != 0u;
        if (two_streams) {
            ctl.fused = false;
            ctl.tev_src = nullptr; ctl.slice_lo = 0u; ctl.slice_hi = 0u;
            ctl.arrive = nullptr; ctl.mt.n_mixers = 0u;
            ctl.ov_heads_counter = s_cmd[2] ? pl.ov_heads + par : nullptr; ctl.ov_heads_target = s_cmd[11];
            ctl.ov_render_counter = pl.ov_render + par;
        } else {
        ctl.fused = true;
        ctl.ov_heads_counter = nullptr; ctl.ov_render_counter = nullptr;
        ctl.arrive = pl.arrive + par; ctl.arrive_target = s_cmd[7];
        ctl.mt = pl.mt;
        ctl.mt.n_mixers = s_cmd[8];
        float *const o = sel == 0u ? pl.out[0] : sel == 1u ? pl.out[1] : pl.out[2];
        if (pl.mt.rows_done != nullptr) {
            const uint32_t rs = s_cmd[10] & 1u;
            ctl.mt.out = rs ? pl.rows_mine[1] : pl.rows_mine[0];
            ctl.mt.rows = rs ? pl.rows[1] : pl.rows[0];
            ctl.mt.rows_done = pl.mt.rows_done + rs;
            ctl.mt.rows_target = s_cmd[9];
            ctl.mt.stereo = 0;
            ctl.mt.done = S2rDone{pl.mt.xmode == 2 ? pl.done_flag + sel : nullptr, s_cmd[3], pl.done_counter + sel};
            ctl.mt.final_out = sel == 0u ? pl.final_out[0] : sel == 1u ? pl.final_out[1] : pl.final_out[2];
            ctl.mt.final_done = S2rDone{pl.final_flag + sel, s_cmd[3], nullptr};
            ctl.mt.final_stereo = stereo;
        } else {
            ctl.mt.out = o;
            ctl.mt.stereo = stereo;
            ctl.mt.done = S2rDone{pl.done_flag + sel, s_cmd[3], pl.done_counter + sel};
            if (s_cmd[12] != 0u && pl.granules != nullptr) { ctl.mt.granules = pl.granules; ctl.mt.granule_tag = s_cmd[3]; }
        }
        }
        if (frames != 0u && frames <= a.p.frames) fill(ctl);
        __syncthreads();
    }
    if (blockIdx.x == 0u && tid == 0u) __hip_atomic_store(pl.exited, pl.launch_id, __ATOMIC_RELAXED, __HIP_MEMORY_SCOPE_SYSTEM);
}

template <int OSC, int SRC, int FILT = 0, bool FMV = false, int NZ = 0, bool AFLAT = false>
__device__ __forceinline__ void chunk_fast(const S2rRenderParams &p, VoiceRegs &r, const EnvRun &ea, const EnvRun &em,
                                           const FlatCache &fc, const OscK &k, uint32_t o_chunk, const float *tab,
                                           const uint64_t *sT, const float *sSin, bool live, uint32_t tile_m0,
                                           float *pv_dst, const FiltCoef *fcoef = nullptr, Filt2 *f2 = nullptr) {
    constexpr bool SMALL = NZ >= 1, ALIGNED = NZ == 2;
    tile_set_base(tile_m0);
    f4 xq[4], bq[4], gq[4], pq[4], iq[4];
    if (SRC == 1) {
        const uint32_t plane = p.tab.plane;
#pragma unroll
        for (int q = 0; q < 4; ++q) {
            xq[q] = load_f4u(tab + 4 * q);
            if (FILT != 0) { bq[q] = load_f4u(tab + plane + 4 * q); gq[q] = load_f4u(tab + 2u * plane + 4 * q); }
            if (FMV) pq[q] = load_f4u(tab + p.tab.fm_plane * plane + 4 * q);
        }
    }
    const double rcp_period = (OSC == S2R_OSC_SINE && !FMV) ? s2r_rcp_f64(k.period) : 0.0;
    r.last = live ? r.last : 0.0f;
    const float ea_slope = live ? ea.s0 : 0.0f, ea_base = live ? ea.s1 : 0.0f, ea_y0 = live ? ea.s2 : 0.0f;
    const float xc0 = live ? fc.xc : 1.0f;
    f4 amp[4], nz[4];
    const float t_chunk = (float)o_chunk;
    const uint32_t o_lo = o_chunk & 0xffffu;
    uint32_t o01 = pk_add_u16(o_lo | (o_lo << 16), 0x00010000u), o23 = pk_add_u16(o01, 0x00020002u);
    const uint32_t seed_pair = (r.seed_rot & 0xffffu) | (r.seed_rot << 16);
    f4 t_small = splat(t_chunk) + (f4){0.0f, 1.0f, 2.0f, 3.0f};
    f4 nzt[4];
    if (ALIGNED) {
        const float *np = p.noise_tab + ((r.seed_rot ^ o_chunk) & 0xffffu);
#pragma unroll
        for (int q = 0; q < 4; ++q) nzt[q] = *reinterpret_cast<const f4 *>(np + 4 * q);
    }
#pragma unroll
    for (int q = 0; q < 4; ++q) {
        f4 t;
        if (ALIGNED) {
            t = t_small;
            t_small = t_small + splat(4.0f);
            nz[q] = nzt[q];
        } else if (SMALL) {
            t = t_small;
            nz[q] = hash_noise4_low16(seed_pair, o01, o23);
            t_small = t_small + splat(4.0f);
            o01 = pk_add_u16(o01, 0x00040004u); o23 = pk_add_u16(o23, 0x00040004u);
        } else {
            const u4 ou = (u4)(o_chunk + 4u * q) + (u4){0u, 1u, 2u, 3u};
            t = __builtin_convertvector(ou, f4);
            nz[q] = hash_noise4(r.seed_rot, t) + splat(p.noise_level);
        }
        if (AFLAT) amp[q] = splat(ea_slope * (t_chunk - ea_base) + ea_y0);
        else amp[q] = splat(ea_slope) * pk_add4(t, splat(-ea_base)) + splat(ea_y0);
        if (SRC == 0) xq[q] = splat(xc0);
        if (SRC == 1 && FMV) {
            const f4 f_osc = pq[q] * splat(r.pitch);
            pq[q] = splat(p.sr) / f_osc;
            iq[q] = splat(1.0f) / pq[q];
        }
        if (SRC == 2) {
            const f4 mod = splat(em.s0) * (t - splat(em.s1)) + splat(em.s2);
            const f4 f_lpf = pow2_sleef_core4(mod * splat(p.amt_lpf)) * splat(p.lpf_freq);
            const f4 num = splat(-2.0f * 3.14159274101257324f) * f_lpf;
            const f4 arg = p.fast_div_sr ? div_const_nocheck4(num, p.sr, p.rcp_sr) : (num / splat(p.sr));
            xq[q] = expf4(arg, sT);
        }
    }
    const uint32_t livemask = live ? 0xffffffffu : 0u;
    f4 outs[4];
#pragma unroll
    for (int q = 0; q < 4; ++q) {
        f4 a0 = splat(1.0f) - xq[q];
        if (SRC == 2 && !live) a0 = splat(0.0f);
        const f4 period = FMV ? pq[q] : splat(k.period), inv_period = FMV ? iq[q] : splat(k.inv_period);
        f4 ph;
        float phc = r.phase;
#pragma unroll
        for (int j = 0; j < 4; ++j) {
            ph[j] = phc;
            phc = __builtin_amdgcn_fractf(phc + inv_period[j]);
        }
        r.phase = phc;
        const f4 x = period * ph;
        f4 osc;
        if (OSC == S2R_OSC_SAW) {
            const f4 ka = FMV ? splat(-2.0f) * inv_period : splat(k.a);
            osc = vfma(ka, x, splat(1.0f));
        } else if (OSC == S2R_OSC_SQUARE) {
            const f4 ka = FMV ? period * splat(0.5f) : splat(k.a);
            const u4 d = (u4)(x - ka);
            osc = -(f4)((d & 0x80000000u) | 0x3f800000u);
        } else if (OSC == S2R_OSC_TRIANGLE) {
            const f4 ka = FMV ? period * splat(0.5f) : splat(k.a);
            const f4 kb = FMV ? splat(-4.0f) * inv_period : splat(k.b), kc = FMV ? splat(4.0f) * inv_period : splat(k.c);
            const f4 first = vfma(kb, x, splat(1.0f)), second = vfma(kc, x - ka, splat(-1.0f));
            const u4 lt = (u4)((i4)(u4)(x - ka) >> 31);
            osc = (f4)(((u4)first & lt) | ((u4)second & ~lt));
        } else {
            osc = sine_quad<FMV>(x, period, rcp_period, sSin);
        }
        const f4 sv = pk_add4(osc + splat(p.osc_gain), nz[q]);
        f4 y;
#pragma unroll
        for (int j = 0; j < 4; ++j) {
            if (FILT == 0) {
                y[j] = __builtin_fmaf(a0[j], sv[j], xq[q][j] * r.last);
                r.last = y[j];
            } else {
                FiltCoef cj = *fcoef;
                if (SRC == 1) { cj.alpha = xq[q][j]; cj.beta = bq[q][j]; cj.gamma = gq[q][j]; }
                y[j] = dsp_filter_apply(FILT, cj, sv[j], *f2);
            }
        }
        f4 out = y * amp[q];
        if (FILT != 0) out = (f4)((u4)out & livemask);
        tile_store4(q, out);
        outs[q] = out;
    }
    if (pv_dst) {
#pragma unroll
        for (int q = 0; q < 4; ++q) *reinterpret_cast<f4u *>(pv_dst + 4 * q) = outs[q];
    }
}

}
```

### synth2_amd/csrc/s2r_render_general.inc

```
#include "s2r_kern_common.h"

namespace {

struct LanePatch {
    int32_t osc_kind;
    float osc_gain, noise_level, lpf_freq, amt_osc, amt_lpf;
    int32_t lpf_kind;
    float lpf_damping;
    S2rEnv amp, mod;
    float sr, rcp_sr;
    S2rTabRef tab;
    uint32_t tab_off;
};

__device__ __forceinline__ LanePatch lane_patch_from_bank(const S2rBankEntry *bank, uint32_t n, uint32_t program, float sr,
                                                          const float *tab_base) {
    const S2rBankEntry e = bank[program < n ? program : 0u];
    LanePatch lp;
    lp.osc_kind = e.osc_kind; lp.osc_gain = e.osc_gain; lp.noise_level = e.noise_level; lp.lpf_freq = e.lpf_freq;
    lp.amt_osc = e.amt_osc; lp.amt_lpf = e.amt_lpf; lp.lpf_kind = e.lpf_kind; lp.lpf_damping = e.lpf_shape;
    lp.amp = e.amp; lp.mod = e.mod; lp.sr = sr; lp.rcp_sr = 0.0f;
    lp.tab.base = (e.tab_valid && tab_base) ? tab_base : nullptr;
    lp.tab_off = e.tab_off;
    lp.tab.plane = e.tab_plane; lp.tab.ad = e.tab_ad; lp.tab.rc = e.tab_rc; lp.tab.rc_t0 = e.tab_rc_t0; lp.tab.ru = e.tab_ru;
// ... 222 lines not shown
    else if (ovh) {
        __shared__ uint32_t s_ok;
        if (tid == 0) { const bool ok = ov_wait(ctl.ov_heads_counter, ctl.ov_heads_target); if (!ok) ov_raise(ctl.fail, 1u); s_ok = ok ? 1u : 0u; }
        __syncthreads();
        if (s_ok == 0u) {
            float *row = ctl.partials + (size_t)blockIdx.x * p.frames_stride;
            for (uint32_t f = 4u * tid; f < p.frames_stride && f < ((ctl.frames + 3u) & ~3u); f += 4u * blockDim.x) ov_store4(row + f, (f4){0.0f, 0.0f, 0.0f, 0.0f});
            if (ctl.ov_render_counter != nullptr) ov_signal(ctl.ov_render_counter);
            return;
        }
    }
    const bool in_range = vi < p.n_voices;
    const uint32_t flags = in_range ? p.v.flags[vi] : 0u;
    bool live = (flags & S2R_VF_STARTED) != 0u;
    LanePatch lp;
    uint32_t program = 0u;
    if constexpr (BANK) {
        program = live ? p.v.program[vi] : 0u;
        lp = lane_patch_from_bank(p.bank, p.bank_size, program, p.sr, p.no_flat_shortcut ? nullptr : p.tab.base);
    } else {
        lp.osc_kind = p.osc_kind; lp.osc_gain = p.osc_gain; lp.noise_level = p.noise_level; lp.lpf_freq = p.lpf_freq;
        lp.amt_osc = p.amt_osc; lp.amt_lpf = p.amt_lpf; lp.lpf_kind = p.lpf_kind; lp.lpf_damping = p.lpf_damping;
        lp.amp = p.amp; lp.mod = p.mod; lp.sr = p.sr; lp.rcp_sr = p.rcp_sr;
        lp.tab = p.tab; lp.tab_off = 0u;
    }
    VoiceRegs r;
    r.pitch = live ? p.v.pitch[vi] : 440.0f;
    r.offset = live ? p.v.offset[vi] : 0u;
    r.release_u = live ? p.v.release[vi] : 0u;
    r.released = live && (flags & S2R_VF_RELEASED) != 0u;
    r.phase = live ? p.v.phase[vi] : 0.0f;
    r.last = live ? p.v.lpf_last[vi] : 0.0f;
    Filt2 f2;
    f2.x1 = live ? p.v.fx1[vi] : 0.0f; f2.x2 = live ? p.v.fx2[vi] : 0.0f;
    f2.y1 = live ? p.v.fy1[vi] : 0.0f; f2.y2 = live ? p.v.fy2[vi] : 0.0f;
    const uint32_t seed = live ? p.v.seed[vi] : 0u;
    r.seed_rot = (seed << 5) | (seed >> 27);
    float osc_z = 0.0f;
    if (OSC == S2R_OSC_ANY) osc_z = live ? p.v.osc_z[vi] : 0.0f;
    auto set_release_thresholds = [&]() {
        const float rf = r.released ? (float)r.release_u : 4294967296.0f;
        r.ro_a = __builtin_fmaxf(rf, BANK ? lp.amp.sus_off : p.amp.sus_off); r.end_a = r.ro_a + (BANK ? lp.amp.R : p.amp.R);
        r.ro_m = __builtin_fmaxf(rf, BANK ? lp.mod.sus_off : p.mod.sus_off); r.end_m = r.ro_m + (BANK ? lp.mod.R : p.mod.R);
    };
    int32_t ev_idx = -1;
    uint32_t ev_frame = 0xffffffffu;
    bool ev_dirty = false, ev_restart = false;
    uint32_t seed_now = seed;
    auto take_releases = [&]() {
        while (ev_idx >= 0) {
            const S2rTimedEvent e = tev_load(ctl.tev, ovh, ev_idx);
            const uint32_t rel = r.offset + e.frame;
            const bool base_ok = r.offset <= (1u << 24) || r.offset >= 0u - ctl.frames;
            if ((e.flags & S2R_EV_RESTART) || !(base_ok && rel <= (1u << 24))) { ev_frame = e.frame; return; }
            if ((e.flags & S2R_EV_RELEASE) && live && !r.released) { r.released = true; r.release_u = rel; }
            ev_dirty = true;
            ev_idx = e.next;
        }
        ev_frame = 0xffffffffu;
    };
    if (TEV && in_range) {
        ev_idx = ovh ? ov_load(ctl.heads + vi) : ctl.heads[vi];
        if (ev_idx >= 0) { if (ovh) ov_store(ctl.heads + vi, (int32_t)-1); else ctl.heads[vi] = -1; take_releases(); }
    }
    set_release_thresholds();

    EnvRun ea = env_stage_at(lp.amp, r.ro_a, r.end_a, (float)r.offset), em = env_stage_at(lp.mod, r.ro_m, r.end_m, (float)r.offset);
    float thr_min = __builtin_fminf(ea.s3, em.s3);
    uint32_t mod_key = 0xffffffffu;
    OscK k = make_osck_any<OSC>(lp.osc_kind, lp.sr / r.pitch);
    float xc = 0.0f;
    FiltCoef fc; fc.alpha = fc.beta = fc.gamma = 0.0f;
    fc.k = lp.lpf_kind >= S2R_FILT_SVF_LP ? 1.0f / lp.lpf_damping : 0.0f;
    __syncthreads();

    const bool wave_live = __ballot(live || ev_idx >= 0) != 0ull;
    const uint32_t x16_frames = ctl.frames & ~(uint32_t)(kChunk - 1);
    const size_t pv_base = (size_t)vi * ctl.frames;
    float *bp = ctl.partials + (size_t)blockIdx.x * p.frames_stride;
    uint32_t buf = 0;
    constexpr bool kFast = !BANK && MAXT == 256;
    const bool fmv = p.amt_osc != 0.0f;
    const bool have_tab = kFast && p.tab.base != nullptr && !p.no_flat_shortcut;
    constexpr bool kBank = BANK && MAXT == 256;
    const bool flat_tab = have_tab && !fmv;
    FiltCoef fc_s = fc, fc_0 = fc;
    if (flat_tab) {
        const float *tb = p.tab.base; const uint32_t pl = p.tab.plane;
        fc_s.alpha = tb[p.tab.sus]; fc_s.beta = tb[pl + p.tab.sus]; fc_s.gamma = tb[2u * pl + p.tab.sus];
        fc_0.alpha = tb[p.tab.end]; fc_0.beta = tb[pl + p.tab.end]; fc_0.gamma = tb[2u * pl + p.tab.end];
    }
    auto end_of_release = [&](float t0) {
        if (ea.s4 == 3.0f && !(t0 < ea.s3)) { ea.s0 = 0.0f; ea.s1 = 0.0f; ea.s2 = 0.0f; ea.s3 = __builtin_inff(); ea.s4 = 4.0f; }
        if (em.s4 == 3.0f && !(t0 < em.s3)) { em.s0 = 0.0f; em.s1 = 0.0f; em.s2 = 0.0f; em.s3 = __builtin_inff(); em.s4 = 4.0f; }
        if (ea.s4 == 2.0f && !(t0 < ea.s3)) { const bool rel = t0 < r.end_a;
            ea.s0 = rel ? lp.amp.slope_rel : 0.0f; ea.s1 = rel ? r.ro_a : 0.0f; ea.s2 = rel ? lp.amp.S : 0.0f;
            ea.s3 = rel ? r.end_a : __builtin_inff(); ea.s4 = rel ? 3.0f : 4.0f; }
        if (em.s4 == 2.0f && !(t0 < em.s3)) { const bool rel = t0 < r.end_m;
            em.s0 = rel ? lp.mod.slope_rel : 0.0f; em.s1 = rel ? r.ro_m : 0.0f; em.s2 = rel ? lp.mod.S : 0.0f;
            em.s3 = rel ? r.end_m : __builtin_inff(); em.s4 = rel ? 3.0f : 4.0f; }
    };
    BankLane bl = make_bank_lane(lp);
    bool wk_dirty = true, wk_ok = false, wk_sine = false, wk_poly = false, wk_fmv = false, wk_dpw = false;
    uint32_t wk_fams = 1u;
    auto classify = [&]() {
        bl = make_bank_lane(lp);
        const uint64_t lm = __ballot(live);
        wk_sine = __ballot(live && lp.osc_kind == S2R_OSC_SINE) != 0ull;
        wk_poly = __ballot(live && lp.osc_kind < S2R_OSC_SINE) != 0ull;
        wk_dpw = OSC == S2R_OSC_ANY && __ballot(live && lp.osc_kind >= S2R_OSC_DPW_SAW && lp.osc_kind <= S2R_OSC_DPW_TRIANGLE) != 0ull;
        wk_ok = lm != 0ull && __ballot(live && !(lp.tab.base != nullptr && lp.osc_kind <= S2R_OSC_DPW_TRIANGLE)) == 0ull &&
                !(wk_dpw && (wk_sine || wk_poly));
        wk_fmv = __ballot(live && lp.amt_osc != 0.0f) != 0ull;
        wk_fams = (__ballot(live && bl.fam == 0u) != 0ull ? 1u : 0u) | (__ballot(live && bl.fam == 1u) != 0ull ? 2u : 0u)
                | (__ballot(live && bl.fam == 2u) != 0ull ? 4u : 0u) | (__ballot(live && bl.fam == 3u) != 0ull ? 8u : 0u);
        wk_dirty = false;
    };

    const uint32_t rf = lane & 15u, rgrp = lane >> 4;
    const float *const tsrc = tile + rf * kTileRow + rgrp * 16u;
    const f4 *const tsrc4 = reinterpret_cast<const f4 *>(tsrc);
    float *const sw_dummy = wave_scratch + lane;
    float *pend_dst = sw_dummy;
    auto tsum = [&]() {
        float tv[16];
#pragma unroll
        for (int q = 0; q < 4; ++q) { const f4 t4 = tsrc4[q]; tv[4 * q] = t4.x; tv[4 * q + 1] = t4.y; tv[4 * q + 2] = t4.z; tv[4 * q + 3] = t4.w; }
        float acc = tv[0];
#pragma unroll
        for (int q = 1; q < 16; ++q) acc += tv[q];
        return acc;
    };
    auto flush_pending = [&]() {
        *pend_dst = tsum();
        pend_dst = sw_dummy;
        __builtin_amdgcn_wave_barrier();
    };
    auto reduce_chunk = [&](uint32_t f_base, uint32_t n_frames) {
        const uint32_t f = lane & 15u, grp = lane >> 4;
        __builtin_amdgcn_wave_barrier();
        if (f < n_frames) {
            const float *src = tile + f * kTileRow + grp * 16u;
            float acc = src[0];
#pragma unroll
            for (int q = 1; q < 16; ++q) acc += src[q];
            sW[(buf * n_groups + wave * GW + grp) * kSuper + f_base + f] = acc;
        }
        __builtin_amdgcn_wave_barrier();
    };
    auto apply_events_at = [&](uint32_t fpos) {
        if (__ballot(ev_frame == fpos) == 0ull) return;
        while (ev_frame == fpos) {
            const S2rTimedEvent e = tev_load(ctl.tev, ovh, ev_idx);
            if (e.flags & S2R_EV_RESTART) {
                r.pitch = e.pitch;
                r.offset = 0u - fpos;
                r.release_u = 0u;
                r.released = (e.flags & S2R_EV_RELEASE) != 0u;
                r.phase = 0.0f; r.last = 0.0f;
                mod_key = 0xffffffffu;
                f2.x1 = f2.x2 = f2.y1 = f2.y2 = 0.0f;
                seed_now = e.seed;
                r.seed_rot = (e.seed << 5) | (e.seed >> 27);
                if constexpr (BANK) { program = e.program; lp = lane_patch_from_bank(p.bank, p.bank_size, program, p.sr, p.no_flat_shortcut ? nullptr : p.tab.base); }
                if (OSC == S2R_OSC_ANY) osc_z = s2r_u2f(S2R_OSC_Z_NONE);
                if constexpr (BANK) fc.k = lp.lpf_kind >= S2R_FILT_SVF_LP ? 1.0f / lp.lpf_damping : 0.0f;
// ... 67 lines not shown
                    }
                    if (run) {
                        run = (uint32_t)__builtin_amdgcn_readfirstlane((int)run);
                        const int first = __builtin_ctzll(__ballot(live));
                        const TabCur cur0 = tab_cursor(lp.tab, em.s4, r.ro_m > lp.mod.sus_off, r.release_u, live);
                        const uint32_t f_off = (uint32_t)__builtin_amdgcn_readlane((int)lp.tab_off, first);
                        const uint32_t f_plane = (uint32_t)__builtin_amdgcn_readlane((int)lp.tab.plane, first);
                        const int32_t f_dead = __builtin_amdgcn_readlane(lp.tab.dead, first);
                        const float *const tbase = p.tab.base + (live ? lp.tab_off : f_off);
                        const uint32_t plane = live ? lp.tab.plane : f_plane;
                        const int32_t cidx = live ? cur0.idx : f_dead;
                        const float period0 = live ? lp.sr / r.pitch : 64.0f;
                        auto loop = [&](auto sine_tag, auto poly_tag, auto fmv_tag, auto fams_tag, auto dpw_tag) {
                            for (uint32_t i = 0; i < run; ++i) {
                                const uint32_t f0 = c16 + i * kChunk;
                                float *pvd = (PV && in_range) ? p.per_voice + pv_base + sc0 + f0 : nullptr;
                                const uint32_t oc = o_chunk + i * kChunk;
                                const float *tp = tbase + (ptrdiff_t)(cidx + (int32_t)(oc & cur0.mask));
                                constexpr bool kDpw = decltype(dpw_tag)::value;
                                const float z_new = chunk_bank<decltype(sine_tag)::value, decltype(poly_tag)::value, decltype(fmv_tag)::value,
                                                               decltype(fams_tag)::value, kDpw>(lp, bl, r, f2, kDpw ? osc_z : 0.0f, ea, period0, oc, tp, plane, sSin, live,
                                                                                                tile_lds, pvd, pend_dst, tsrc4);
                                if (kDpw) osc_z = z_new;
                                __builtin_amdgcn_wave_barrier();
                                pend_dst = sW + (buf * n_groups + wave * GW + rgrp) * kSuper + rf + f0;
                            }
                        };
                        const std::true_type T; const std::false_type F;
                        auto pick_osc = [&](auto fmv_tag, auto fams_tag) {
                            if (wk_dpw) loop(F, F, fmv_tag, fams_tag, T);
                            else if (wk_sine && wk_poly) loop(T, T, fmv_tag, fams_tag, F);
                            else if (wk_sine) loop(T, F, fmv_tag, fams_tag, F);
                            else loop(F, T, fmv_tag, fams_tag, F);
                        };
                        auto pick_fmv = [&](auto fams_tag) { if (wk_fmv) pick_osc(T, fams_tag); else pick_osc(F, fams_tag); };
                        switch (wk_fams) {
#define S2R_FAMS_CASE(N) case N: pick_fmv(std::integral_constant<int, N>{}); break;
                        S2R_FAMS_CASE(1) S2R_FAMS_CASE(2) S2R_FAMS_CASE(3) S2R_FAMS_CASE(4) S2R_FAMS_CASE(5) S2R_FAMS_CASE(6)
                        S2R_FAMS_CASE(7) S2R_FAMS_CASE(8) S2R_FAMS_CASE(9) S2R_FAMS_CASE(10) S2R_FAMS_CASE(11) S2R_FAMS_CASE(12)
                        S2R_FAMS_CASE(13) S2R_FAMS_CASE(14)
#undef S2R_FAMS_CASE
                        default: pick_fmv(std::integral_constant<int, 15>{}); break;
                        }
                        mod_key = 0xffffffffu;
                        c16 += (run - 1u) * kChunk;
                        continue;
                    }
                }
                const bool flat = calm && __ballot(live && em.s0 != 0.0f) == 0ull;
                if (flat) {
                    if (flat_tab) {
                        const bool zero = em.s2 == 0.0f;
                        fc.alpha = zero ? fc_0.alpha : fc_s.alpha; fc.beta = zero ? fc_0.beta : fc_s.beta; fc.gamma = zero ? fc_0.gamma : fc_s.gamma;
                        mod_key = 0xffffffffu;
                    } else refresh(live ? env_value(em, (float)(r.offset + sc0 + c16)) : 0.0f);
                }
                const bool tab_chunk = have_tab && !flat && calm && __ballot(r.offset + sc0 + c16 + kChunk > (1u << 24)) == 0ull;
                if (kFast && calm && (flat || tab_chunk)) {
                    const uint32_t left = (n_x16 - c16) / kChunk;
                    const uint32_t o_chunk = r.offset + sc0 + c16;
                    auto clear_for = [&](uint32_t n) {
                        return __ballot(!((float)(o_chunk + n * kChunk - 1u) < thr_min)) == 0ull;
                    };
                    uint32_t run = 1u;
                    {
                        const float q = ((thr_min - (float)o_chunk) + 1.0f) * 0.0625f;
                        float nf = __builtin_ceilf(q) - 1.0f;
                        nf = __builtin_fminf(__builtin_fmaxf(nf, 1.0f), (float)left);
                        uint32_t n = (uint32_t)nf;
                        if (TEV) { const uint32_t ne = (ev_frame - (sc0 + c16)) >> 4; n = ne < n ? ne : n; }
                        n = wave_min_u32(n);
                        if (n > 1u && clear_for(n)) run = n;
                    }
                    if (tab_chunk && __ballot(o_chunk + run * kChunk > (1u << 24)) != 0ull) run = 1u;
                    if (__ballot(!(((tab_chunk && fmv) ? (!live || lp.sr >= r.pitch * 0x1p-115f) : (k.period >= 0x1p-126f && k.period < __builtin_inff())) && r.phase >= 0.0f && r.phase < 1.0f)) != 0ull) run = 0u;
                    if (run) {
                        run = (uint32_t)__builtin_amdgcn_readfirstlane((int)run);
                        FlatCache fcx; fcx.xc = xc; fcx.k = k;
                        const FiltCoef fcc = fc;
                        const TabCur cur = tab_cursor(p.tab, em.s4, r.ro_m > lp.mod.sus_off, r.release_u, live);
                        const bool nz_aligned = p.noise_tab != nullptr && p.noise_level == 0.0f &&
                                                __ballot(o_chunk + run * kChunk > (1u << 24) || ((o_chunk | r.seed_rot) & 15u) != 0u) == 0ull;
                        const bool amp_flat = nz_aligned && __ballot(live && ea.s0 != 0.0f) == 0ull;
                        auto run_chunks = [&](auto filt_tag) {
                            constexpr int FILT = decltype(filt_tag)::value;
                            constexpr int O = OSC == S2R_OSC_ANY ? 0 : OSC;
                            auto loop = [&](auto src_tag, auto fmv_tag, auto nz_tag, auto aflat_tag) {
                                constexpr int SRC = decltype(src_tag)::value;
                                constexpr bool FMV = decltype(fmv_tag)::value;
                                constexpr int NZ = decltype(nz_tag)::value;
                                constexpr bool AFLAT = decltype(aflat_tag)::value;
                                for (uint32_t i = 0; i < run; ++i) {
                                    const uint32_t f0 = c16 + i * kChunk;
                                    float *pvd = (PV && in_range) ? p.per_voice + pv_base + sc0 + f0 : nullptr;
                                    const uint32_t oc = o_chunk + i * kChunk;
                                    const float *tp = p.tab.base + (ptrdiff_t)(cur.idx + (int32_t)(oc & cur.mask));
                                    *pend_dst = tsum();
                                    chunk_fast<O, SRC, FILT, FMV, NZ, AFLAT>(p, r, ea, em, fcx, k, oc, tp, sT, sSin, live, tile_lds, pvd, &fcc, &f2);
                                    __builtin_amdgcn_wave_barrier();
                                    pend_dst = sW + (buf * n_groups + wave * GW + rgrp) * kSuper + rf + f0;
                                }
                            };
                            using T = std::true_type; using F = std::false_type;
                            using S0 = std::integral_constant<int, 0>; using S1 = std::integral_constant<int, 1>;
                            using N0 = std::integral_constant<int, 0>; using N2 = std::integral_constant<int, 2>;
                            if (tab_chunk && fmv) loop(S1{}, T{}, N0{}, F{});
                            else if (!tab_chunk) { if (amp_flat) loop(S0{}, F{}, N2{}, T{}); else if (nz_aligned) loop(S0{}, F{}, N2{}, F{}); else loop(S0{}, F{}, N0{}, F{}); }
                            else { if (amp_flat) loop(S1{}, F{}, N2{}, T{}); else if (nz_aligned) loop(S1{}, F{}, N2{}, F{}); else loop(S1{}, F{}, N0{}, F{}); }
                        };
                        switch (lp.lpf_kind) {
                        case S2R_FILT_LP1: run_chunks(std::integral_constant<int, S2R_FILT_LP1>{}); break;
                        case S2R_FILT_HP1: run_chunks(std::integral_constant<int, S2R_FILT_HP1>{}); break;
                        case S2R_FILT_LP2: run_chunks(std::integral_constant<int, S2R_FILT_LP2>{}); break;
                        case S2R_FILT_HP2: run_chunks(std::integral_constant<int, S2R_FILT_HP2>{}); break;
                        case S2R_FILT_BP2: run_chunks(std::integral_constant<int, S2R_FILT_BP2>{}); break;
                        case S2R_FILT_SVF_LP: run_chunks(std::integral_constant<int, S2R_FILT_SVF_LP>{}); break;
                        case S2R_FILT_SVF_BP: run_chunks(std::integral_constant<int, S2R_FILT_SVF_BP>{}); break;
                        case S2R_FILT_SVF_HP: run_chunks(std::integral_constant<int, S2R_FILT_SVF_HP>{}); break;
                        default: break;
                        }
                        c16 += (run - 1u) * kChunk;
                        continue;
                    }
                }
                flush_pending();
                for (uint32_t j = 0; j < kChunk; ++j) {
                    const uint32_t oi = r.offset + sc0 + c16 + j;
                    const float t = (float)oi;
                    if (!calm && !(t < thr_min)) {
                        ea = env_stage_at(lp.amp, r.ro_a, r.end_a, t);
                        em = env_stage_at(lp.mod, r.ro_m, r.end_m, t);
                        thr_min = __builtin_fminf(ea.s3, em.s3);
                    }
                    const float amp = env_value(ea, t);
                    const float mod = env_value(em, t);
                    if (!flat) refresh(mod);
                    const float nz = hash_noise(r.seed_rot, t) + lp.noise_level;
                    const float ph = r.phase;
                    r.phase = s2r_fmod1(ph + k.inv_period);
                    const float off = __builtin_fmaf(k.period, ph, 0.0f);
                    float osc;
                    if (OSC == S2R_OSC_ANY && lp.osc_kind >= S2R_OSC_DPW_SAW) osc = dpw_value(lp.osc_kind, k, off, osc_z);
                    else osc = osc_value_any<OSC>(lp.osc_kind, k, off, sSin);
                    const float smp = (osc + lp.osc_gain) + nz;
                    float y;
                    if (lp.lpf_kind == S2R_FILT_ONEPOLE) y = lpf_apply(xc, smp, r.last);
                    else y = dsp_filter_apply(lp.lpf_kind, fc, smp, f2);
                    const float out = live ? y * amp : 0.0f;
                    if (PV && in_range) p.per_voice[pv_base + sc0 + c16 + j] = out;
                    tile[j * kTileRow + lane] = out;
                }
                reduce_chunk(c16, kChunk);
            }
            flush_pending();
            if (n_x16 < n_sc) {
                if (TEV) apply_events_at(sc0 + n_x16);
                for (uint32_t i = n_x16; i < n_sc; ++i) {
                    float out;
                    if (lp.lpf_kind == S2R_FILT_ONEPOLE) out = frame_sisd<OSC, false, LanePatch>(lp, r, r.offset + sc0 + i, sT, sSin, nullptr, &osc_z);
                    else out = frame_sisd<OSC, true, LanePatch>(lp, r, r.offset + sc0 + i, sT, sSin, &f2, &osc_z);
                    out = live ? out : 0.0f;
                    if (PV && in_range) p.per_voice[pv_base + sc0 + i] = out;
                    tile[(i - n_x16) * kTileRow + lane] = out;
                }
                reduce_chunk(n_x16, n_sc - n_x16);
            }
        } else {
            for (uint32_t i = lane; i < GW * kSuper; i += 64u)
                sW[(buf * n_groups + wave * GW + i / kSuper) * kSuper + (i % kSuper)] = 0.0f;
            if (PV && in_range) for (uint32_t i = 0; i < n_sc; ++i) p.per_voice[pv_base + sc0 + i] = 0.0f;
        }
        __syncthreads();
        combine_groups(p, ctl.done, sW + (size_t)buf * n_groups * kSuper, n_groups, kSuper, n_sc, sc0, bp + sc0, tid, blockDim.x, nullptr, 0u, ctl.fused || ctl.ov_render_counter != nullptr);
        buf ^= 1u;
    }

    if (live) {
        const uint32_t o = r.offset;
        p.v.offset[vi] = (!ev_dirty && o > 0xffffffffu - ctl.frames) ? 0xffffffffu : o + ctl.frames;
        p.v.phase[vi] = r.phase;
        p.v.lpf_last[vi] = r.last;
        p.v.fx1[vi] = f2.x1; p.v.fx2[vi] = f2.x2; p.v.fy1[vi] = f2.y1; p.v.fy2[vi] = f2.y2;
        if (OSC == S2R_OSC_ANY) p.v.osc_z[vi] = osc_z;
        else if (ev_restart) p.v.osc_z[vi] = s2r_u2f(S2R_OSC_Z_NONE);
        if (ev_dirty) {
            p.v.pitch[vi] = r.pitch;
            p.v.release[vi] = r.release_u;
            p.v.flags[vi] = S2R_VF_STARTED | (r.released ? S2R_VF_RELEASED : 0u);
            p.v.seed[vi] = seed_now;
            if (BANK) p.v.program[vi] = program;
        }
// ... 77 lines not shown
```

### synth2_amd/csrc/s2r_render_onepole.inc

```
#include "s2r_kern_common.h"

namespace {

template <int OSC, bool FM, int MODE, int MAXT>
__device__ __forceinline__ void render_fill(const S2rRenderArgs &a, const FillCtl &ctl) {
    const S2rRenderParams &p = a.p;
    constexpr bool PV = MODE == 1;
    constexpr bool TEV = MODE == 2;
    const uint32_t kSuper = p.super_frames;
    __shared__ uint64_t sT[S2R_EXP2F_N];
    __shared__ __attribute__((aligned(8))) float sSin[OSC == S2R_OSC_SINE ? 2048 : 2];
    extern __shared__ __attribute__((aligned(16))) float s_dyn[];
    __shared__ uint32_t s_word;

    const uint32_t tid = threadIdx.x;
    const uint32_t lane = tid & 63u, wave = tid >> 6, n_waves = blockDim.x >> 6;
    constexpr uint32_t VW = 64;
    constexpr uint32_t GW = VW / 16;
    const uint32_t n_groups = n_waves * GW;
    float *const sW = s_dyn;
    constexpr uint32_t kTile = kChunk * kTileRow;
    const uint32_t sw_floats = s2r_sw_buffers(p.frames, kSuper) * n_groups * kSuper;
    float *const tile = s_dyn + sw_floats + wave * kTile;
    float *const wave_scratch = s_dyn + sw_floats + n_waves * kTile + wave * 64u;
// ... 38 lines not shown
            return;
        }
    }
    auto tev_at = [&](int32_t i) -> S2rTimedEvent { return tev_load(ctl.tev, ovh, i); };
    uint32_t flags = 0u, w_offset = 0u, w_release = 0u, w_seed = 0u;
    float w_pitch = 440.0f, w_phase = 0.0f, w_last = 0.0f;
    int32_t ev_idx = -1;
    if (in_range) {
        flags = p.v.flags[vi];
        w_pitch = p.v.pitch[vi]; w_offset = p.v.offset[vi]; w_release = p.v.release[vi];
        w_phase = p.v.phase[vi]; w_last = p.v.lpf_last[vi]; w_seed = p.v.seed[vi];
        if (TEV) ev_idx = ovh ? ov_load(ctl.heads + vi) : ctl.heads[vi];
    }
    bool live = (flags & S2R_VF_STARTED) != 0u;
    uint32_t ev_frame = 0xffffffffu;
    S2rTimedEvent ev_next{};
    bool ev_dirty = false, ev_restart = false;
    if (TEV && ev_idx >= 0) {
        ev_next = tev_at(ev_idx);
        ev_frame = ev_next.frame;
        if (ovh) ov_store(ctl.heads + vi, (int32_t)-1); else ctl.heads[vi] = -1;
    }
    VoiceRegs r;
    r.pitch = live ? w_pitch : 440.0f;
    r.offset = live ? w_offset : 0u;
    r.release_u = live ? w_release : 0u;
    r.released = live && (flags & S2R_VF_RELEASED) != 0u;
    r.phase = live ? w_phase : 0.0f;
    r.last = live ? w_last : 0.0f;
    uint32_t seed = live ? w_seed : 0u;
    uint32_t program_now = 0u;
    if (TEV && ev_frame == 0u) {
        const S2rTimedEvent e = ev_next;
        if (e.flags & S2R_EV_RESTART) {
            r.pitch = e.pitch; r.offset = 0u; r.release_u = 0u;
            r.released = (e.flags & S2R_EV_RELEASE) != 0u;
            r.phase = 0.0f; r.last = 0.0f;
            { const S2rTimedEvent er = tev_at(ev_idx); seed = er.seed; program_now = er.program; }
            live = true; ev_restart = true;
        } else if ((e.flags & S2R_EV_RELEASE) && live && !r.released) {
            r.released = true;
            r.release_u = r.offset;
        }
        ev_dirty = true;
        ev_idx = e.next;
        ev_frame = 0xffffffffu;
        if (ev_idx >= 0) { ev_next = tev_at(ev_idx); ev_frame = ev_next.frame; }
    }
    bool took_release = false;
    auto take_releases = [&]() {
        while (ev_idx >= 0 && !(ev_next.flags & S2R_EV_RESTART)) {
            const uint32_t rel = r.offset + ev_next.frame;
            const bool base_ok = r.offset <= (1u << 24) || r.offset >= 0u - ctl.frames;
            if (!(base_ok && rel <= (1u << 24))) break;
            if ((ev_next.flags & S2R_EV_RELEASE) && live && !r.released) {
                r.released = true;
                r.release_u = rel;
                took_release = true;
            }
            ev_dirty = true;
            ev_idx = ev_next.next;
            ev_frame = 0xffffffffu;
            if (ev_idx >= 0) { ev_next = tev_at(ev_idx); ev_frame = ev_next.frame; }
        }
    };
    if (TEV) take_releases();
    r.seed_rot = (seed << 5) | (seed >> 27);

    const float rel_f = r.released ? (float)r.release_u : 4294967296.0f;
    r.ro_a = __builtin_fmaxf(rel_f, p.amp.sus_off); r.end_a = r.ro_a + p.amp.R;
    r.ro_m = __builtin_fmaxf(rel_f, p.mod.sus_off); r.end_m = r.ro_m + p.mod.R;

    OscK k_const = make_osck<OSC>(p.sr / (1.0f * r.pitch));
    uint32_t seed_now = seed;

    EnvRun ea = env_stage_at(p.amp, r.ro_a, r.end_a, (float)r.offset);
    EnvRun em = env_stage_at(p.mod, r.ro_m, r.end_m, (float)r.offset);
    float thr_min = __builtin_fminf(ea.s3, em.s3);
    FlatCache fc;
    fc.xc = 0.0f; fc.k = k_const;

    __syncthreads();
    const bool have_tab = p.tab.base != nullptr && !p.no_flat_shortcut;
    FlatConsts fcc = (have_tab && (!FM || p.tab.fm_plane != 0u)) ? flat_consts_from_tables<OSC, FM>(p, r.pitch) : make_flat_consts<OSC, FM>(p, r.pitch, sT);
    fc = refresh_flat<OSC, FM>(fcc, em, fc);

    const bool wave_live = __ballot(live || ev_idx >= 0) != 0ull;
    bool wave_events = TEV && __ballot(ev_idx >= 0) != 0ull;
    const uint32_t x16_frames = ctl.frames & ~(uint32_t)(kChunk - 1);
    const bool fast_ok = __ballot(!(r.phase >= 0.0f && r.phase < 1.0f)) == 0ull &&
        (FM || __ballot(!(k_const.period >= 0x1p-126f && k_const.period < __builtin_inff())) == 0ull);
    const size_t pv_base = (size_t)vi * ctl.frames;
    float *bp = ctl.partials + (size_t)blockIdx.x * p.frames_stride;
    uint32_t buf = 0;

    auto reduce_chunk = [&](uint32_t f_base, uint32_t n_frames) {
        const uint32_t f = lane & 15u, grp = lane >> 4;
        __builtin_amdgcn_wave_barrier();
        if (f < n_frames) {
            const float *src = tile + f * kTileRow + grp * 16u;
            float acc = src[0];
#pragma unroll
            for (int k = 1; k < 16; ++k) acc += src[k];
            sW[(buf * n_groups + wave * GW + grp) * kSuper + f_base + f] = acc;
        }
        __builtin_amdgcn_wave_barrier();
    };

    bool w_flat = false, w_aflat = false, w_aligned = false, w_small = false;
    auto reclassify_stages = [&]() {
        w_flat = !p.no_flat_shortcut && __ballot(live && em.s0 != 0.0f) == 0ull &&
                 (!FM || __ballot(!(fc.k.period >= 0x1p-126f && fc.k.period < __builtin_inff())) == 0ull);
        w_aflat = __ballot(live && ea.s0 != 0.0f) == 0ull;
    };
    auto reclassify = [&]() {
        reclassify_stages();
        w_aligned = p.noise_tab != nullptr && __ballot(((r.offset | r.seed_rot) & 15u) != 0u) == 0ull;
        w_small = __ballot(r.offset + ctl.frames > (1u << 24)) == 0ull;
    };
    reclassify();
    stamp(1);

    auto apply_events_lane = [&](uint32_t fpos) -> bool {
        bool restarted = false, released_now = false;
        took_release = false;
        while (ev_frame == fpos) {
            const S2rTimedEvent e = ev_next;
            if (e.flags & S2R_EV_RESTART) {
                r.pitch = e.pitch;
                r.offset = 0u - fpos;
                r.release_u = 0u;
                r.released = (e.flags & S2R_EV_RELEASE) != 0u;
                r.phase = 0.0f; r.last = 0.0f;
                const S2rTimedEvent er = tev_at(ev_idx);
                seed_now = er.seed;
                r.seed_rot = (seed_now << 5) | (seed_now >> 27);
                program_now = er.program;
                live = true; ev_restart = true; restarted = true;
                k_const = make_osck<OSC>(p.sr / (1.0f * r.pitch));
            } else if ((e.flags & S2R_EV_RELEASE) && live && !r.released) {
                r.released = true;
                r.release_u = r.offset + fpos;
                released_now = true;
            }
            ev_dirty = true;
            ev_idx = e.next;
            ev_frame = 0xffffffffu;
            if (ev_idx >= 0) { ev_next = tev_at(ev_idx); ev_frame = ev_next.frame; }
            take_releases();
        }
        const float rf = r.released ? (float)r.release_u : 4294967296.0f;
        r.ro_a = __builtin_fmaxf(rf, p.amp.sus_off); r.end_a = r.ro_a + p.amp.R;
        r.ro_m = __builtin_fmaxf(rf, p.mod.sus_off); r.end_m = r.ro_m + p.mod.R;
        const float t0 = (float)(r.offset + fpos);
        if (restarted) {
            if (FM) {
                const FlatConsts n = (have_tab && p.tab.fm_plane != 0u) ? flat_consts_from_tables<OSC, FM>(p, r.pitch) : make_flat_consts<OSC, FM>(p, r.pitch, sT);
                fcc.k_s = n.k_s; fcc.k_0 = n.k_0;
            }
            ea = env_stage_at(p.amp, r.ro_a, r.end_a, t0);
            em = env_stage_at(p.mod, r.ro_m, r.end_m, t0);
        } else if (released_now) {
            if (ea.s4 == 2.0f) { const bool rel = t0 < r.end_a;
                ea.s0 = rel ? p.amp.slope_rel : 0.0f; ea.s1 = rel ? r.ro_a : 0.0f; ea.s2 = rel ? p.amp.S : 0.0f;
                ea.s3 = rel ? r.end_a : __builtin_inff(); ea.s4 = rel ? 3.0f : 4.0f; }
            if (em.s4 == 2.0f) { const bool rel = t0 < r.end_m;
// ... 8 lines not shown
        fc = refresh_flat<OSC, FM>(fcc, em, fc);
        return restarted;
    };

    auto apply_events_at = [&](uint32_t fpos) {
        if (!wave_events || __ballot(ev_frame == fpos) == 0ull) return;
        dbg_events += (uint32_t)__builtin_popcountll(__ballot(ev_frame == fpos));
        bool restarted = false;
        if (ev_frame == fpos) restarted = apply_events_lane(fpos);
        if (__ballot(restarted) != 0ull) {
            w_aligned = p.noise_tab != nullptr && __ballot(((r.offset | r.seed_rot) & 15u) != 0u) == 0ull;
            w_small = __ballot(r.offset + ctl.frames > (1u << 24)) == 0ull;
        }
        wave_events = __ballot(ev_idx >= 0) != 0ull;
        w_flat = !p.no_flat_shortcut && __ballot(live && em.s0 != 0.0f) == 0ull &&
                 (!FM || __ballot(!(fc.k.period >= 0x1p-126f && fc.k.period < __builtin_inff())) == 0ull);
        w_aflat = __ballot(live && ea.s0 != 0.0f) == 0ull;
    };

    auto end_of_release = [&](float t0) {
        if (ea.s4 == 3.0f && !(t0 < ea.s3)) { ea.s0 = 0.0f; ea.s1 = 0.0f; ea.s2 = 0.0f; ea.s3 = __builtin_inff(); ea.s4 = 4.0f; }
        if (em.s4 == 3.0f && !(t0 < em.s3)) { em.s0 = 0.0f; em.s1 = 0.0f; em.s2 = 0.0f; em.s3 = __builtin_inff(); em.s4 = 4.0f; }
        if (ea.s4 == 2.0f && !(t0 < ea.s3)) { const bool rel = t0 < r.end_a;
            ea.s0 = rel ? p.amp.slope_rel : 0.0f; ea.s1 = rel ? r.ro_a : 0.0f; ea.s2 = rel ? p.amp.S : 0.0f;
            ea.s3 = rel ? r.end_a : __builtin_inff(); ea.s4 = rel ? 3.0f : 4.0f; }
        if (em.s4 == 2.0f && !(t0 < em.s3)) { const bool rel = t0 < r.end_m;
            em.s0 = rel ? p.mod.slope_rel : 0.0f; em.s1 = rel ? r.ro_m : 0.0f; em.s2 = rel ? p.mod.S : 0.0f;
            em.s3 = rel ? r.end_m : __builtin_inff(); em.s4 = rel ? 3.0f : 4.0f; }
    };

    const uint32_t rf = lane & 15u, rgrp = lane >> 4;
    const float *const tsrc = tile + rf * kTileRow + rgrp * 16u;
    const f4 *const tsrc4 = reinterpret_cast<const f4 *>(tsrc);
    float *const sw_dummy = wave_scratch + lane;
    float *pend_dst = sw_dummy;
    auto tsum = [&]() {
        float tv[16];
#pragma unroll
        for (int q = 0; q < 4; ++q) { const f4 t4 = tsrc4[q]; tv[4 * q] = t4.x; tv[4 * q + 1] = t4.y; tv[4 * q + 2] = t4.z; tv[4 * q + 3] = t4.w; }
        float acc = tv[0];
#pragma unroll
        for (int q = 1; q < 16; ++q) acc += tv[q];
        return acc;
    };
    auto flush_pending = [&]() {
        *pend_dst = tsum();
        pend_dst = sw_dummy;
        __builtin_amdgcn_wave_barrier();
    };

    bool dense_stay = false;
    for (uint32_t sc0 = 0; sc0 < ctl.frames; sc0 += kSuper) {
        const uint32_t n_sc = (ctl.frames - sc0 < kSuper) ? (ctl.frames - sc0) : kSuper;
        const uint32_t n_x16 = (x16_frames > sc0) ? ((x16_frames - sc0 < n_sc) ? (x16_frames - sc0) : n_sc) : 0u;
        if (wave_live) {
            for (uint32_t c16 = 0; c16 < n_x16; c16 += kChunk) {
                const unsigned long long dbg_tt0 = S2R_DBG_NOW();
                if (TEV) apply_events_at(sc0 + c16);
                const bool dense = TEV && wave_events && fast_ok && have_tab && w_small && w_aligned && p.noise_level == 0.0f &&
                                   (!FM || __ballot(live && !(p.sr >= r.pitch * 0x1p-115f)) == 0ull) &&
                                   (dense_stay || wave_min_u32((ev_frame - (sc0 + c16)) >> 4) <= 2u);
                dbg_t_top += S2R_DBG_NOW() - dbg_tt0;
                if (dense) {
                    bool inside = false;
                    bool idle_exit = false;
                    constexpr uint32_t kNoRel = 0xffffffffu;
                    uint32_t pend_rel = kNoRel;
                    auto commit_plain = [&]() {
                        if (pend_rel != kNoRel) {
                            if ((ev_next.flags & S2R_EV_RELEASE) && live && !r.released) {
                                r.released = true;
                                r.release_u = pend_rel;
                                const float rf = (float)pend_rel;
                                r.ro_a = __builtin_fmaxf(rf, p.amp.sus_off); r.end_a = r.ro_a + p.amp.R;
                                r.ro_m = __builtin_fmaxf(rf, p.mod.sus_off); r.end_m = r.ro_m + p.mod.R;
                            }
                            ev_dirty = true; ev_idx = -1;
                            pend_rel = kNoRel;
                        }
                    };
                    auto plain_now = [&]() { return !(ev_next.flags & S2R_EV_RESTART) && ev_next.next < 0 && ea.s4 <= 1.0f && em.s4 <= 1.0f; };
                    bool plain = plain_now();
                    TabCur cur = tab_cursor(p.tab, em.s4, r.ro_m > p.mod.sus_off, r.release_u, live);
                    const unsigned long long dbg_td0 = S2R_DBG_NOW();
                    while (c16 < n_x16 && wave_events && !idle_exit) {
                        {
                            const uint32_t fpos = sc0 + c16;
                            bool lane_bad = false;
                            const bool hit = ev_frame == fpos;
                            commit_plain();
                            if (hit) {
                                dbg_events += 1u;
                                if (apply_events_lane(fpos)) lane_bad = ((r.offset | r.seed_rot) & 15u) != 0u || r.offset + ctl.frames > (1u << 24);
                            }
                            const uint32_t oc = r.offset + fpos;
                            const float t0 = (float)oc;
                            end_of_release(t0);
                            thr_min = __builtin_fminf(ea.s3, em.s3);
                            if (!(t0 < thr_min)) {
                                ea = env_stage_at(p.amp, r.ro_a, r.end_a, t0);
                                em = env_stage_at(p.mod, r.ro_m, r.end_m, t0);
                                thr_min = __builtin_fminf(ea.s3, em.s3);
                            }
                            fc = refresh_flat<OSC, FM>(fcc, em, fc);
                            cur = tab_cursor(p.tab, em.s4, r.ro_m > p.mod.sus_off, r.release_u, live);
                            plain = plain_now();
                            wave_events = __ballot(ev_idx >= 0) != 0ull;
                            const bool bad_align = __ballot(lane_bad) != 0ull;
                            inside = __ballot(!((float)(oc + (kChunk - 1u)) < thr_min)) != 0ull;
                            if (bad_align) { w_aligned = false; w_small = false; }
                            if (inside || bad_align) break;
                        }
                        for (;;) {
                            const uint32_t fpos = sc0 + c16;
                            const uint32_t oc = r.offset + fpos;
                            ++dbg_dense;
                            *pend_dst = tsum();
                            float *pvd = (PV && in_range) ? p.per_voice + pv_base + fpos : nullptr;
                            const float *tp = p.tab.base + (ptrdiff_t)(cur.idx + (int32_t)(oc & cur.mask));
                            chunk_fast<OSC, 1, 0, FM, 2, false>(p, r, ea, em, fc, FM ? fc.k : k_const, oc, tp, sT, sSin, live, tile_lds, pvd);
                            __builtin_amdgcn_wave_barrier();
                            pend_dst = sW + (buf * n_groups + wave * GW + rgrp) * kSuper + rf + c16;
                            c16 += kChunk;
                            if (c16 >= n_x16) break;
                            const uint32_t fnext = fpos + kChunk, onext = oc + kChunk;
                            const bool hit = ev_frame == fnext;
                            if (__ballot((hit && !plain) || !((float)(onext + (kChunk - 1u)) < thr_min)) != 0ull) break;
                            pend_rel = hit ? onext : pend_rel;
                            ev_frame = hit ? 0xffffffffu : ev_frame;
                            if ((c16 & 0x30u) == 0x30u) {
                                const uint64_t pending = __ballot(ev_frame != 0xffffffffu);
                                if (pending == 0ull) { idle_exit = true; break; }
                                if (__builtin_popcountll(pending) <= 4) {
                                    const uint32_t nxt = wave_min_u32(ev_frame);
                                    if (((nxt - fnext) >> 4) > 8u) { idle_exit = true; break; }
                                }
                            }
                        }
                    }
                    commit_plain();
                    wave_events = __ballot(ev_idx >= 0) != 0ull;
                    dense_stay = wave_events && !idle_exit && !inside && c16 >= n_x16;
                    dbg_t_dense += S2R_DBG_NOW() - dbg_td0;
                    reclassify();
                    if (c16 >= n_x16) break;
                    if (!inside) { c16 -= kChunk; continue; }
                }
                const unsigned long long dbg_ts0 = S2R_DBG_NOW();
                const uint32_t o_chunk = r.offset + sc0 + c16;
                if (fast_ok) {
                    const uint32_t left = (n_x16 - c16) / kChunk;
                    auto clear_for = [&](uint32_t n) {
                        bool bad = !((float)(o_chunk + n * kChunk - 1u) < thr_min);
                        if (TEV) bad = bad || ev_frame < sc0 + c16 + n * kChunk;
                        return __ballot(bad) == 0ull;
                    };
                    auto pick_run = [&]() -> uint32_t {
                        const float q = ((thr_min - (float)o_chunk) + 1.0f) * 0.0625f;
                        float nf = __builtin_ceilf(q) - 1.0f;
                        nf = __builtin_fminf(__builtin_fmaxf(nf, 0.0f), (float)left);
                        uint32_t n = (uint32_t)nf;
                        if (TEV) { const uint32_t ne = (ev_frame - (sc0 + c16)) >> 4; n = ne < n ? ne : n; }
                        n = wave_min_u32(n);
                        if (n == 0u) return 0u;
                        if (clear_for(n)) return n;
                        return (n > 1u && clear_for(1u)) ? 1u : 0u;
                    };
                    {
                        const float t0 = (float)o_chunk;
                        if (__ballot(!(t0 < thr_min)) != 0ull) {
                            end_of_release(t0);
                            thr_min = __builtin_fminf(ea.s3, em.s3);
                            if (!(t0 < thr_min)) {
                                ea = env_stage_at(p.amp, r.ro_a, r.end_a, t0);
                                em = env_stage_at(p.mod, r.ro_m, r.end_m, t0);
                                thr_min = __builtin_fminf(ea.s3, em.s3);
                            }
                            fc = refresh_flat<OSC, FM>(fcc, em, fc);
                            reclassify_stages();
                        }
                    }
                    const unsigned long long dbg_ts1 = S2R_DBG_NOW();
                    dbg_t_casc += dbg_ts1 - dbg_ts0;
                    uint32_t run = pick_run();
                    dbg_t_pick1 += S2R_DBG_NOW() - dbg_ts1;
                    bool flat = false, tab_ok = false, offs_small = false;
                    if (run) {
                        run = (uint32_t)__builtin_amdgcn_readfirstlane((int)run);
                        offs_small = w_small || __ballot(o_chunk + run * kChunk > (1u << 24)) == 0ull;
                        flat = w_flat;
                        tab_ok = !flat && have_tab && offs_small;
                        if (FM && !flat && !tab_ok) run = 0;
                        if (FM && !flat && __ballot(live && !(p.sr >= r.pitch * 0x1p-115f)) != 0ull) run = 0;
                    }
                    if (run) {
                        ++dbg_runs; dbg_runchunks += run;
                        const unsigned long long dbg_tr0 = S2R_DBG_NOW();
                        dbg_t_sel += dbg_tr0 - dbg_ts0;
                        float *const sw_row = sW + (buf * n_groups + wave * GW + rgrp) * kSuper + rf;
                        const TabCur cur = tab_cursor(p.tab, em.s4, r.ro_m > p.mod.sus_off, r.release_u, live);
                        auto run_chunks = [&](auto src_tag, auto nz_tag, auto aflat_tag) {
                            constexpr int SRC = decltype(src_tag)::value;
                            constexpr int NZ = decltype(nz_tag)::value;
                            constexpr bool AFLAT = decltype(aflat_tag)::value;
                            for (uint32_t i = 0; i < run; ++i) {
                                const uint32_t f0 = c16 + i * kChunk;
                                *pend_dst = tsum();
                                float *pvd = (PV && in_range) ? p.per_voice + pv_base + sc0 + f0 : nullptr;
                                const uint32_t oc = o_chunk + i * kChunk;
                                const float *tp = p.tab.base + (ptrdiff_t)(cur.idx + (int32_t)(oc & cur.mask));
                                chunk_fast<OSC, SRC, 0, (FM && SRC == 1), NZ, AFLAT>(p, r, ea, em, fc, FM ? fc.k : k_const, oc, tp, sT, sSin, live,
                                                                              tile_lds, pvd);
                                __builtin_amdgcn_wave_barrier();
                                pend_dst = sw_row + f0;
                            }
                        };
                        const bool small = p.noise_level == 0.0f && offs_small;
                        const bool aligned = small && w_aligned && ((sc0 + c16) & 15u) == 0u;
                        const bool aflat = aligned && w_aflat;
                        using T = std::true_type; using F = std::false_type;
                        using N0 = std::integral_constant<int, 0>; using N1 = std::integral_constant<int, 1>; using N2 = std::integral_constant<int, 2>;
                        if (tab_ok) {
                            if (aflat) run_chunks(N1{}, N2{}, T{});
                            else if (aligned) run_chunks(N1{}, N2{}, F{});
                            else if (small) run_chunks(N1{}, N1{}, F{});
                            else run_chunks(N1{}, N0{}, F{});
                        } else if (flat) {
                            if (aflat) run_chunks(N0{}, N2{}, T{});
                            else if (aligned) run_chunks(N0{}, N2{}, F{});
                            else if (small) run_chunks(N0{}, N1{}, F{});
                            else run_chunks(N0{}, N0{}, F{});
                        } else if (!FM) {
                            if (aligned) run_chunks(N2{}, N2{}, F{});
                            else if (small) run_chunks(N2{}, N1{}, F{});
                            else run_chunks(N2{}, N0{}, F{});
                        }
                        c16 += (run - 1u) * kChunk;
                        dbg_t_run += S2R_DBG_NOW() - dbg_tr0;
                        continue;
                    }
                }
                flush_pending();
                ++dbg_general;
                for (uint32_t g = c16; g < c16 + kChunk; g += kP) {
                    FrameCF4 cf; OscK4 kf;
                    closed_form_x4<OSC, FM>(p, r, ea, em, thr_min, fc, fcc, r.offset + sc0 + g, sT, cf, kf);
                    f4 out4;
#pragma unroll
                    for (int j = 0; j < kP; ++j) {
                        FrameCF c1; c1.amp = cf.amp[j]; c1.xc = cf.xc[j]; c1.nz = cf.nz[j];
                        OscK k1 = k_const;
                        if (FM) { k1.period = kf.period[j]; k1.inv_period = kf.inv_period[j];
                                  k1.a = kf.a[j]; k1.b = kf.b[j]; k1.c = kf.c[j]; }
                        const float o = recur_x16<OSC>(p, r, c1, k1, sSin);
                        out4[j] = live ? o : 0.0f;
                    }
                    if (PV) { if (in_range) {
                        float *dst = p.per_voice + pv_base + sc0 + g;
                        dst[0] = out4.x; dst[1] = out4.y; dst[2] = out4.z; dst[3] = out4.w; } }
                    float *trow = tile + (g & 15u) * kTileRow + lane;
                    trow[0 * kTileRow] = out4.x; trow[1 * kTileRow] = out4.y;
                    trow[2 * kTileRow] = out4.z; trow[3 * kTileRow] = out4.w;
                }
                reduce_chunk(c16, kChunk);
                reclassify();
            }
            flush_pending();
            if (n_x16 < n_sc) {
                if (TEV) apply_events_at(sc0 + n_x16);
                for (uint32_t i = n_x16; i < n_sc; ++i) {
                    float out = frame_sisd<OSC>(p, r, r.offset + sc0 + i, sT, sSin);
                    out = live ? out : 0.0f;
                    if (PV) { if (in_range) p.per_voice[pv_base + sc0 + i] = out; }
                    tile[(i - n_x16) * kTileRow + lane] = out;
                }
                reduce_chunk(n_x16, n_sc - n_x16);
            }
        } else {
            for (uint32_t i = lane; i < GW * kSuper; i += 64u)
                sW[(buf * n_groups + wave * GW + i / kSuper) * kSuper + (i % kSuper)] = 0.0f;
            if (PV) { if (in_range) for (uint32_t i = 0; i < n_sc; ++i) p.per_voice[pv_base + sc0 + i] = 0.0f; }
        }
        stamp(2u + 2u * stamp_k);
        __syncthreads();
        combine_groups(p, ctl.done, sW + (size_t)buf * n_groups * kSuper, n_groups, kSuper, n_sc, sc0, bp + sc0, tid, blockDim.x, ctl.granules, ctl.granule_tag, ctl.fused || ctl.ov_render_counter != nullptr);
        buf ^= 1u;
        stamp(3u + 2u * stamp_k);
        ++stamp_k;
    }

    if (live) {
        const uint32_t o = r.offset;
        p.v.offset[vi] = (!ev_dirty && o > 0xffffffffu - ctl.frames) ? 0xffffffffu : o + ctl.frames;
        p.v.phase[vi] = r.phase;
        p.v.lpf_last[vi] = r.last;
        if (ev_dirty) {
            p.v.pitch[vi] = r.pitch;
            p.v.release[vi] = r.release_u;
            p.v.flags[vi] = S2R_VF_STARTED | (r.released ? S2R_VF_RELEASED : 0u);
            p.v.seed[vi] = seed_now;
            if (ev_restart) {
                p.v.fx1[vi] = 0.0f; p.v.fx2[vi] = 0.0f; p.v.fy1[vi] = 0.0f; p.v.fy2[vi] = 0.0f;
                p.v.osc_z[vi] = s2r_u2f(S2R_OSC_Z_NONE);
                p.v.program[vi] = program_now;
            }
        }
    }
    if (p.direct_out && ctl.granules == nullptr) signal_done(ctl.done, 1u);
    if (ctl.ov_render_counter != nullptr) ov_signal(ctl.ov_render_counter);
#if defined(S2R_STAMPS)
    if (p.stamps && lane == 0) p.stamps[(size_t)(vi >> 6) * 16u + 8u] = __builtin_amdgcn_s_memrealtime();
    if (ctl.fused) fused_tail(p, ctl, sW, &s_word, p.stamps ? p.stamps + (size_t)(vi >> 6) * 16u : nullptr);
#else
    if (ctl.fused) fused_tail(p, ctl, sW, &s_word);
#endif
#if defined(S2R_STAMPS)
    if (p.stamps && lane == 0) { unsigned long long *d = p.stamps + (size_t)(vi >> 6) * 16u; d[11] = dbg_events; d[12] = (unsigned long long)dbg_dense | ((dbg_t_pick1 & 0x3fffffull) << 20) | ((dbg_t_casc & 0x3fffffull) << 42); d[13] = (dbg_t_top << 32) | (dbg_t_sel & 0xffffffffull); d[14] = dbg_runs;
        d[10] = ((unsigned long long)dbg_runchunks << 48) | ((dbg_t_dense & 0xffffffull) << 24) | (dbg_t_run & 0xffffffull); }
// ... 150 lines not shown
```

Measured before the change: 1665 billion.

## Precompute amplitude envelope table and load per-frame amplitude in aligned chunks

Adds a device-built amplitude-envelope lookup table, laid out like the existing modulation coefficient table, in the same allocation. Aligned, non-flat chunks in the onepole and general render paths now read four f4 amplitude vectors from this table instead of computing the linear envelope per frame. The intent is to remove per-frame envelope arithmetic from the hot chunk loop. In exchange it adds extra global or cached memory loads per chunk, more template instantiations, and an env var S2R_AMP_TAB=0 to turn it off.

```diff
diff --git a/synth2_amd/csrc/s2r_aux.hip b/synth2_amd/csrc/s2r_aux.hip
--- a/synth2_amd/csrc/s2r_aux.hip
+++ b/synth2_amd/csrc/s2r_aux.hip
@@ -46,6 +46,29 @@
     if (b.fm_plane) b.base[(size_t)b.fm_plane * b.plane + i] = dead ? 1.0f : s2r_pow2_sleef_core(mod * b.amt_osc);
 }
 
+__global__ void __launch_bounds__(256) s2r_amp_table_kernel(const S2rTabBuild b) {
+    const uint32_t i = blockIdx.x * blockDim.x + threadIdx.x;
+    if (i >= b.n_entries) return;
+    const S2rEnv &e = b.mod;
+    float amp;
+    if (i < b.n_ad) {
+        const float t = (float)i;
+        const EnvRun s = env_stage_at(e, __builtin_inff(), __builtin_inff(), t);
+        amp = env_value(s, t);
+    } else if (i < b.n_ad + b.n_rel) {
+        const float t = (float)(b.rc_t0 + (i - b.n_ad));
+        amp = e.slope_rel * (t - e.sus_off) + e.S;
+    } else if (i < b.n_ad + 2u * b.n_rel) {
+        const float d = (float)(i - b.n_ad - b.n_rel);
+        amp = e.slope_rel * d + e.S;
+    } else if (i < b.n_ad + 2u * b.n_rel + 16u) {
+        amp = 0.0f * 1.0f + e.S;
+    } else {
+        amp = 0.0f;
+    }
+    b.base[i] = amp;
+}
+
 __global__ void __launch_bounds__(256) s2r_noise_table_kernel(float *t) {
     const uint32_t x = blockIdx.x * blockDim.x + threadIdx.x;
     const float f = (float)((x * 0x79b9u) & 0xffffu) * 0x1p-16f;
@@ -184,6 +207,12 @@
     return hipGetLastError();
 }
 
+hipError_t s2r_launch_amp_table(const S2rTabBuild &b, hipStream_t stream) {
+    if (b.n_entries == 0) return hipErrorInvalidValue;
+    hipLaunchKernelGGL(s2r_amp_table_kernel, dim3((b.n_entries + 255u) / 256u), dim3(256), 0, stream, b);
+    return hipGetLastError();
+}
+
 hipError_t s2r_launch_noise_table(float *table_65536, hipStream_t stream) {
     hipLaunchKernelGGL(s2r_noise_table_kernel, dim3(65536 / 256), dim3(256), 0, stream, table_65536);
     return hipGetLastError();
diff --git a/synth2_amd/csrc/s2r_device.h b/synth2_amd/csrc/s2r_device.h
--- a/synth2_amd/csrc/s2r_device.h
+++ b/synth2_amd/csrc/s2r_device.h
@@ -114,13 +114,16 @@
     const float *sin_table;
     const float *noise_tab;
     S2rTabRef tab;
+    const float *atab;
     const S2rTimedEvent *tev;
     int32_t *voice_ev_head;
     unsigned long long *stamps;
     unsigned long long *timeline;
     uint32_t tl_slot;
+    uint32_t atab_rc_t0;
     const S2rBankEntry *bank;
     uint32_t bank_size;
+    uint32_t atab_n_rel;
     const uint32_t *ov_heads_counter;
     uint32_t ov_heads_target;
     uint32_t *ov_render_counter;
@@ -132,6 +135,16 @@
     uint32_t arrive_target;
     S2rMixTail mt;
 };
+
+__host__ __device__ inline S2rTabRef s2r_tab_ref(const float *base, uint32_t rc_t0, uint32_t n_rel) {
+    S2rTabRef t{};
+    const uint32_t n_ad = rc_t0 + 1u + S2R_TAB_PAD;
+    t.base = base;
+    t.ad = 0; t.rc = (int32_t)n_ad; t.rc_t0 = rc_t0; t.ru = (int32_t)(n_ad + n_rel);
+    t.sus = (int32_t)(n_ad + 2u * n_rel); t.end = t.sus + 16; t.dead = t.sus + 32;
+    return t;
+}
+__host__ __device__ inline S2rTabRef s2r_amp_tab_ref(const S2rRenderParams &p) { return s2r_tab_ref(p.atab, p.atab_rc_t0, p.atab_n_rel); }
 
 struct S2rVoiceEvent {
     uint32_t voice;
@@ -243,6 +256,7 @@
 };
 
 hipError_t s2r_launch_tables(const S2rTabBuild &b, hipStream_t stream);
+hipError_t s2r_launch_amp_table(const S2rTabBuild &b, hipStream_t stream);
 hipError_t s2r_launch_noise_table(float *table_65536, hipStream_t stream);
 hipError_t s2r_launch_resident(const S2rRenderArgs &a, const S2rResident &rs, uint32_t block_voices, hipStream_t stream);
 hipError_t s2r_launch_render(const S2rRenderArgs &a, uint32_t block_voices, hipStream_t stream);
diff --git a/synth2_amd/csrc/s2r_host.cpp b/synth2_amd/csrc/s2r_host.cpp
--- a/synth2_amd/csrc/s2r_host.cpp
+++ b/synth2_amd/csrc/s2r_host.cpp
@@ -198,6 +198,7 @@
     float *per_voice_dev = nullptr; size_t per_voice_cap = 0;
     float *tab_dev = nullptr; size_t tab_cap = 0;
     S2rTabRef tab{};
+    const float *atab = nullptr; uint32_t atab_rc_t0 = 0, atab_n_rel = 0;
     bool tab_dirty = true; uint32_t tab_rate = 0;
     float *bank_tab_dev = nullptr; size_t bank_tab_cap = 0;
     unsigned long long *stamps_dev = nullptr;
@@ -494,15 +495,20 @@
     if (!tables_wanted(s)) { return S2R_OK; }
     if (!s->tab_dirty && s->tab_rate == sample_rate) return S2R_OK;
     s->tab = S2rTabRef{};
+    s->atab = nullptr; s->atab_rc_t0 = 0; s->atab_n_rel = 0;
     s->tab_dirty = false; s->tab_rate = sample_rate;
-    S2rTabBuild b{};
-    if (!plan_tables(p.mod, b)) return S2R_OK;
+    S2rTabBuild b{}, ab{};
+    const bool have_coef = plan_tables(p.mod, b);
+    static const bool amp_off = [] { const char *e = std::getenv("S2R_AMP_TAB"); return e && e[0] == '0'; }();
+    const bool have_amp = !amp_off && plan_tables(p.amp, ab);
+    if (!have_coef && !have_amp) return S2R_OK;
     b.lpf_freq = p.lpf_freq; b.amt_lpf = p.amt_lpf; b.amt_osc = p.amt_osc; b.sr = p.sr; b.rcp_sr = p.rcp_sr;
     b.fast_div_sr = p.fast_div_sr; b.lpf_kind = p.lpf_kind; b.lpf_damping = p.lpf_damping;
     const bool onepole = p.lpf_kind == S2R_FILT_ONEPOLE;
     const uint32_t n_planes = (onepole ? 2u : 3u) + (p.amt_osc != 0.0f ? 1u : 0u);
     b.fm_plane = p.amt_osc != 0.0f ? (onepole ? 2u : 3u) : 0u;
-    const size_t need = (size_t)b.plane * n_planes;
+    const size_t coef_floats = have_coef ? (size_t)b.plane * n_planes : 0;
+    const size_t need = coef_floats + (have_amp ? (size_t)ab.plane : 0);
     if (need > s->tab_cap) {
         S2R_HIP(s, hipStreamSynchronize(stream));
         S2R_HIP(s, hipStreamSynchronize(s->stream));
@@ -510,13 +516,17 @@
         S2R_HIP(s, hipMalloc((void **)&s->tab_dev, need * sizeof(float)));
         s->tab_cap = need;
     }
-    b.base = s->tab_dev;
-    S2R_HIP(s, s2r_launch_tables(b, stream));
-    S2rTabRef &t = s->tab;
-    t.base = s->tab_dev; t.plane = b.plane;
-    t.ad = 0; t.rc = (int32_t)b.n_ad; t.rc_t0 = b.rc_t0; t.ru = (int32_t)(b.n_ad + b.n_rel);
-    t.sus = (int32_t)(b.n_ad + 2u * b.n_rel); t.end = t.sus + 16; t.dead = t.sus + 32;
-    t.fm_plane = b.fm_plane;
+    if (have_coef) {
+        b.base = s->tab_dev;
+        S2R_HIP(s, s2r_launch_tables(b, stream));
+        s->tab = s2r_tab_ref(s->tab_dev, b.rc_t0, b.n_rel);
+        s->tab.plane = b.plane; s->tab.fm_plane = b.fm_plane;
+    }
+    if (have_amp) {
+        ab.base = s->tab_dev + coef_floats;
+        S2R_HIP(s, s2r_launch_amp_table(ab, stream));
+        s->atab = ab.base; s->atab_rc_t0 = ab.rc_t0; s->atab_n_rel = ab.n_rel;
+    }
     return S2R_OK;
 }
 
@@ -729,7 +739,7 @@
     { int rc = ensure_bank(s, sample_rate, stream, &bank_kernel); if (rc != S2R_OK) return rc; }
     p = make_params(s, frames, sample_rate);
     { int rc = ensure_tables(s, p, sample_rate, stream); if (rc != S2R_OK) return rc; }
-    if (tables_wanted(s)) p.tab = s->tab;
+    if (tables_wanted(s)) { p.tab = s->tab; p.atab = s->atab; p.atab_rc_t0 = s->atab_rc_t0; p.atab_n_rel = s->atab_n_rel; }
     else if (bank_kernel) { p.tab = S2rTabRef{}; p.tab.base = s->bank_tab_dev; }
     p.stamps = s->stamps_dev;
     if (s->timeline_dev && s->timeline_n < s->timeline_cap) { p.timeline = s->timeline_dev; p.tl_slot = s->timeline_n++; }
@@ -877,7 +887,7 @@
     { int rc = ensure_bank(s, sample_rate, s->stream, &bank_kernel); if (rc != S2R_OK) return rc; }
     p = make_params(s, s->cfg.max_frames, sample_rate);
     { int rc = ensure_tables(s, p, sample_rate, s->stream); if (rc != S2R_OK) return rc; }
-    if (tables_wanted(s)) p.tab = s->tab;
+    if (tables_wanted(s)) { p.tab = s->tab; p.atab = s->atab; p.atab_rc_t0 = s->atab_rc_t0; p.atab_n_rel = s->atab_n_rel; }
     else if (bank_kernel) { p.tab = S2rTabRef{}; p.tab.base = s->bank_tab_dev; }
     p.voice_ev_head = s->voice_ev_head;
     p.stamps = s->stamps_dev;
@@ -1025,7 +1035,7 @@
         int rc = ensure_tables(s, p, sample_rate, stream);
         if (rc != S2R_OK) return rc;
     }
-    if (tables_wanted(s)) p.tab = s->tab;
+    if (tables_wanted(s)) { p.tab = s->tab; p.atab = s->atab; p.atab_rc_t0 = s->atab_rc_t0; p.atab_n_rel = s->atab_n_rel; }
     else if (bank_kernel) { p.tab = S2rTabRef{}; p.tab.base = s->bank_tab_dev; }
     p.stamps = s->stamps_dev;
     if (s->timeline_dev && s->timeline_n < s->timeline_cap) { p.timeline = s->timeline_dev; p.tl_slot = s->timeline_n++; }
@@ -1281,7 +1291,7 @@
     S2rRenderParams &p = a.p;
     p = make_params(s, s->cfg.max_frames, sample_rate);
     { int rc = ensure_tables(s, p, sample_rate, s->stream); if (rc != S2R_OK) return rc; }
-    if (tables_wanted(s)) p.tab = s->tab;
+    if (tables_wanted(s)) { p.tab = s->tab; p.atab = s->atab; p.atab_rc_t0 = s->atab_rc_t0; p.atab_n_rel = s->atab_n_rel; }
     p.voice_ev_head = s->voice_ev_head;
     p.direct_out = s->out_host_dev; p.direct_stereo = stereo ? 1 : 0;
     p.stamps = s->stamps_dev;
diff --git a/synth2_amd/csrc/s2r_kern_common.h b/synth2_amd/csrc/s2r_kern_common.h
--- a/synth2_amd/csrc/s2r_kern_common.h
+++ b/synth2_amd/csrc/s2r_kern_common.h
@@ -1062,12 +1062,14 @@
     if (blockIdx.x == 0u && tid == 0u) __hip_atomic_store(pl.exited, pl.launch_id, __ATOMIC_RELAXED, __HIP_MEMORY_SCOPE_SYSTEM);
 }
 
-template <int OSC, int SRC, int FILT = 0, bool FMV = false, int NZ = 0, bool AFLAT = false>
+template <int OSC, int SRC, int FILT = 0, bool FMV = false, int NZ = 0, bool AFLAT = false, bool ATAB = false>
 __device__ __forceinline__ void chunk_fast(const S2rRenderParams &p, VoiceRegs &r, const EnvRun &ea, const EnvRun &em,
                                            const FlatCache &fc, const OscK &k, uint32_t o_chunk, const float *tab,
                                            const uint64_t *sT, const float *sSin, bool live, uint32_t tile_m0,
-                                           float *pv_dst, const FiltCoef *fcoef = nullptr, Filt2 *f2 = nullptr) {
+                                           float *pv_dst, const FiltCoef *fcoef = nullptr, Filt2 *f2 = nullptr,
+                                           const float *atab = nullptr) {
     constexpr bool SMALL = NZ >= 1, ALIGNED = NZ == 2;
+    static_assert(!ATAB || (ALIGNED && !AFLAT), "the amplitude plane serves the aligned chunk's per-frame amplitude");
     tile_set_base(tile_m0);
     f4 xq[4], bq[4], gq[4], pq[4], iq[4];
     if (SRC == 1) {
@@ -1079,11 +1081,15 @@
             if (FMV) pq[q] = load_f4u(tab + p.tab.fm_plane * plane + 4 * q);
         }
     }
+    f4 amp[4], nz[4];
+    if (ATAB) {
+#pragma unroll
+        for (int q = 0; q < 4; ++q) amp[q] = load_f4u(atab + 4 * q);
+    }
     const double rcp_period = (OSC == S2R_OSC_SINE && !FMV) ? s2r_rcp_f64(k.period) : 0.0;
     r.last = live ? r.last : 0.0f;
     const float ea_slope = live ? ea.s0 : 0.0f, ea_base = live ? ea.s1 : 0.0f, ea_y0 = live ? ea.s2 : 0.0f;
     const float xc0 = live ? fc.xc : 1.0f;
-    f4 amp[4], nz[4];
     const float t_chunk = (float)o_chunk;
     const uint32_t o_lo = o_chunk & 0xffffu;
     uint32_t o01 = pk_add_u16(o_lo | (o_lo << 16), 0x00010000u), o23 = pk_add_u16(o01, 0x00020002u);
@@ -1112,7 +1118,8 @@
             t = __builtin_convertvector(ou, f4);
             nz[q] = hash_noise4(r.seed_rot, t) + splat(p.noise_level);
         }
-        if (AFLAT) amp[q] = splat(ea_slope * (t_chunk - ea_base) + ea_y0);
+        if (ATAB) {}
+        else if (AFLAT) amp[q] = splat(ea_slope * (t_chunk - ea_base) + ea_y0);
         else amp[q] = splat(ea_slope) * pk_add4(t, splat(-ea_base)) + splat(ea_y0);
         if (SRC == 0) xq[q] = splat(xc0);
         if (SRC == 1 && FMV) {
diff --git a/synth2_amd/csrc/s2r_render_general.inc b/synth2_amd/csrc/s2r_render_general.inc
--- a/synth2_amd/csrc/s2r_render_general.inc
+++ b/synth2_amd/csrc/s2r_render_general.inc
@@ -328,6 +328,7 @@
     constexpr bool kFast = !BANK && MAXT == 256;
     const bool fmv = p.amt_osc != 0.0f;
     const bool have_tab = kFast && p.tab.base != nullptr && !p.no_flat_shortcut;
+    const bool have_atab = kFast && p.atab != nullptr && !p.no_flat_shortcut;
     constexpr bool kBank = BANK && MAXT == 256;
     const bool flat_tab = have_tab && !fmv;
     FiltCoef fc_s = fc, fc_0 = fc;
@@ -561,10 +562,13 @@
                         const bool nz_aligned = p.noise_tab != nullptr && p.noise_level == 0.0f &&
                                                 __ballot(o_chunk + run * kChunk > (1u << 24) || ((o_chunk | r.seed_rot) & 15u) != 0u) == 0ull;
                         const bool amp_flat = nz_aligned && __ballot(live && ea.s0 != 0.0f) == 0ull;
+                        const bool amp_tab = nz_aligned && !amp_flat && have_atab;
+                        const TabCur acur = tab_cursor(s2r_amp_tab_ref(p), ea.s4, r.ro_a > lp.amp.sus_off, r.release_u, live);
                         auto run_chunks = [&](auto filt_tag) {
                             constexpr int FILT = decltype(filt_tag)::value;
                             constexpr int O = OSC == S2R_OSC_ANY ? 0 : OSC;
-                            auto loop = [&](auto src_tag, auto fmv_tag, auto nz_tag, auto aflat_tag) {
+                            auto loop = [&](auto src_tag, auto fmv_tag, auto nz_tag, auto aflat_tag, auto atab_tag) {
+                                constexpr bool ATAB = decltype(atab_tag)::value;
                                 constexpr int SRC = decltype(src_tag)::value;
                                 constexpr bool FMV = decltype(fmv_tag)::value;
                                 constexpr int NZ = decltype(nz_tag)::value;
@@ -575,7 +579,8 @@
                                     const uint32_t oc = o_chunk + i * kChunk;
                                     const float *tp = p.tab.base + (ptrdiff_t)(cur.idx + (int32_t)(oc & cur.mask));
                                     *pend_dst = tsum();
-                                    chunk_fast<O, SRC, FILT, FMV, NZ, AFLAT>(p, r, ea, em, fcx, k, oc, tp, sT, sSin, live, tile_lds, pvd, &fcc, &f2);
+                                    const float *ap = ATAB ? p.atab + (ptrdiff_t)(acur.idx + (int32_t)(oc & acur.mask)) : nullptr;
+                                    chunk_fast<O, SRC, FILT, FMV, NZ, AFLAT, ATAB>(p, r, ea, em, fcx, k, oc, tp, sT, sSin, live, tile_lds, pvd, &fcc, &f2, ap);
                                     __builtin_amdgcn_wave_barrier();
                                     pend_dst = sW + (buf * n_groups + wave * GW + rgrp) * kSuper + rf + f0;
                                 }
@@ -583,9 +588,14 @@
                             using T = std::true_type; using F = std::false_type;
                             using S0 = std::integral_constant<int, 0>; using S1 = std::integral_constant<int, 1>;
                             using N0 = std::integral_constant<int, 0>; using N2 = std::integral_constant<int, 2>;
-                            if (tab_chunk && fmv) loop(S1{}, T{}, N0{}, F{});
-                            else if (!tab_chunk) { if (amp_flat) loop(S0{}, F{}, N2{}, T{}); else if (nz_aligned) loop(S0{}, F{}, N2{}, F{}); else loop(S0{}, F{}, N0{}, F{}); }
-                            else { if (amp_flat) loop(S1{}, F{}, N2{}, T{}); else if (nz_aligned) loop(S1{}, F{}, N2{}, F{}); else loop(S1{}, F{}, N0{}, F{}); }
+                            if (tab_chunk && fmv) loop(S1{}, T{}, N0{}, F{}, F{});
+                            else if (!tab_chunk) {
+                                if (amp_flat) loop(S0{}, F{}, N2{}, T{}, F{}); else if (amp_tab) loop(S0{}, F{}, N2{}, F{}, T{});
+                                else if (nz_aligned) loop(S0{}, F{}, N2{}, F{}, F{}); else loop(S0{}, F{}, N0{}, F{}, F{});
+                            } else {
+                                if (amp_flat) loop(S1{}, F{}, N2{}, T{}, F{}); else if (amp_tab) loop(S1{}, F{}, N2{}, F{}, T{});
+                                else if (nz_aligned) loop(S1{}, F{}, N2{}, F{}, F{}); else loop(S1{}, F{}, N0{}, F{}, F{});
+                            }
                         };
                         switch (lp.lpf_kind) {
                         case S2R_FILT_LP1: run_chunks(std::integral_constant<int, S2R_FILT_LP1>{}); break;
diff --git a/synth2_amd/csrc/s2r_render_onepole.inc b/synth2_amd/csrc/s2r_render_onepole.inc
--- a/synth2_amd/csrc/s2r_render_onepole.inc
+++ b/synth2_amd/csrc/s2r_render_onepole.inc
@@ -144,6 +144,8 @@
 
     __syncthreads();
     const bool have_tab = p.tab.base != nullptr && !p.no_flat_shortcut;
+    const bool have_atab = p.atab != nullptr && !p.no_flat_shortcut;
+    const S2rTabRef atab_ref = s2r_amp_tab_ref(p);
     FlatConsts fcc = (have_tab && (!FM || p.tab.fm_plane != 0u)) ? flat_consts_from_tables<OSC, FM>(p, r.pitch) : make_flat_consts<OSC, FM>(p, r.pitch, sT);
     fc = refresh_flat<OSC, FM>(fcc, em, fc);
 
@@ -318,6 +320,7 @@
                     auto plain_now = [&]() { return !(ev_next.flags & S2R_EV_RESTART) && ev_next.next < 0 && ea.s4 <= 1.0f && em.s4 <= 1.0f; };
                     bool plain = plain_now();
                     TabCur cur = tab_cursor(p.tab, em.s4, r.ro_m > p.mod.sus_off, r.release_u, live);
+                    TabCur acur = tab_cursor(atab_ref, ea.s4, r.ro_a > p.amp.sus_off, r.release_u, live);
                     const unsigned long long dbg_td0 = S2R_DBG_NOW();
                     while (c16 < n_x16 && wave_events && !idle_exit) {
                         {
@@ -340,6 +343,7 @@
                             }
                             fc = refresh_flat<OSC, FM>(fcc, em, fc);
                             cur = tab_cursor(p.tab, em.s4, r.ro_m > p.mod.sus_off, r.release_u, live);
+                            acur = tab_cursor(atab_ref, ea.s4, r.ro_a > p.amp.sus_off, r.release_u, live);
                             plain = plain_now();
                             wave_events = __ballot(ev_idx >= 0) != 0ull;
                             const bool bad_align = __ballot(lane_bad) != 0ull;
@@ -351,10 +355,17 @@
                             const uint32_t fpos = sc0 + c16;
                             const uint32_t oc = r.offset + fpos;
                             ++dbg_dense;
-                            *pend_dst = tsum();
                             float *pvd = (PV && in_range) ? p.per_voice + pv_base + fpos : nullptr;
                             const float *tp = p.tab.base + (ptrdiff_t)(cur.idx + (int32_t)(oc & cur.mask));
-                            chunk_fast<OSC, 1, 0, FM, 2, false>(p, r, ea, em, fc, FM ? fc.k : k_const, oc, tp, sT, sSin, live, tile_lds, pvd);
+                            if (have_atab) {
+                                const float *ap = p.atab + (ptrdiff_t)(acur.idx + (int32_t)(oc & acur.mask));
+                                *pend_dst = tsum();
+                                chunk_fast<OSC, 1, 0, FM, 2, false, true>(p, r, ea, em, fc, FM ? fc.k : k_const, oc, tp, sT, sSin, live, tile_lds, pvd,
+                                                                          nullptr, nullptr, ap);
+                            } else {
+                                *pend_dst = tsum();
+                                chunk_fast<OSC, 1, 0, FM, 2, false>(p, r, ea, em, fc, FM ? fc.k : k_const, oc, tp, sT, sSin, live, tile_lds, pvd);
+                            }
                             __builtin_amdgcn_wave_barrier();
                             pend_dst = sW + (buf * n_groups + wave * GW + rgrp) * kSuper + rf + c16;
                             c16 += kChunk;
@@ -435,18 +446,21 @@
                         dbg_t_sel += dbg_tr0 - dbg_ts0;
                         float *const sw_row = sW + (buf * n_groups + wave * GW + rgrp) * kSuper + rf;
                         const TabCur cur = tab_cursor(p.tab, em.s4, r.ro_m > p.mod.sus_off, r.release_u, live);
-                        auto run_chunks = [&](auto src_tag, auto nz_tag, auto aflat_tag) {
+                        const TabCur acur = tab_cursor(atab_ref, ea.s4, r.ro_a > p.amp.sus_off, r.release_u, live);
+                        auto run_chunks = [&](auto src_tag, auto nz_tag, auto aflat_tag, auto atab_tag) {
                             constexpr int SRC = decltype(src_tag)::value;
                             constexpr int NZ = decltype(nz_tag)::value;
                             constexpr bool AFLAT = decltype(aflat_tag)::value;
+                            constexpr bool ATAB = decltype(atab_tag)::value;
                             for (uint32_t i = 0; i < run; ++i) {
                                 const uint32_t f0 = c16 + i * kChunk;
                                 *pend_dst = tsum();
                                 float *pvd = (PV && in_range) ? p.per_voice + pv_base + sc0 + f0 : nullptr;
                                 const uint32_t oc = o_chunk + i * kChunk;
                                 const float *tp = p.tab.base + (ptrdiff_t)(cur.idx + (int32_t)(oc & cur.mask));
-                                chunk_fast<OSC, SRC, 0, (FM && SRC == 1), NZ, AFLAT>(p, r, ea, em, fc, FM ? fc.k : k_const, oc, tp, sT, sSin, live,
-                                                                              tile_lds, pvd);
+                                const float *ap = ATAB ? p.atab + (ptrdiff_t)(acur.idx + (int32_t)(oc & acur.mask)) : nullptr;
+                                chunk_fast<OSC, SRC, 0, (FM && SRC == 1), NZ, AFLAT, ATAB>(p, r, ea, em, fc, FM ? fc.k : k_const, oc, tp, sT, sSin, live,
+                                                                                    tile_lds, pvd, nullptr, nullptr, ap);
                                 __builtin_amdgcn_wave_barrier();
                                 pend_dst = sw_row + f0;
                             }
@@ -454,22 +468,26 @@
                         const bool small = p.noise_level == 0.0f && offs_small;
                         const bool aligned = small && w_aligned && ((sc0 + c16) & 15u) == 0u;
                         const bool aflat = aligned && w_aflat;
+                        const bool atab = aligned && have_atab;
                         using T = std::true_type; using F = std::false_type;
                         using N0 = std::integral_constant<int, 0>; using N1 = std::integral_constant<int, 1>; using N2 = std::integral_constant<int, 2>;
                         if (tab_ok) {
-                            if (aflat) run_chunks(N1{}, N2{}, T{});
-                            else if (aligned) run_chunks(N1{}, N2{}, F{});
-                            else if (small) run_chunks(N1{}, N1{}, F{});
-                            else run_chunks(N1{}, N0{}, F{});
+                            if (aflat) run_chunks(N1{}, N2{}, T{}, F{});
+                            else if (atab) run_chunks(N1{}, N2{}, F{}, T{});
+                            else if (aligned) run_chunks(N1{}, N2{}, F{}, F{});
+                            else if (small) run_chunks(N1{}, N1{}, F{}, F{});
+                            else run_chunks(N1{}, N0{}, F{}, F{});
                         } else if (flat) {
-                            if (aflat) run_chunks(N0{}, N2{}, T{});
-                            else if (aligned) run_chunks(N0{}, N2{}, F{});
-                            else if (small) run_chunks(N0{}, N1{}, F{});
-                            else run_chunks(N0{}, N0{}, F{});
+                            if (aflat) run_chunks(N0{}, N2{}, T{}, F{});
+                            else if (atab) run_chunks(N0{}, N2{}, F{}, T{});
+                            else if (aligned) run_chunks(N0{}, N2{}, F{}, F{});
+                            else if (small) run_chunks(N0{}, N1{}, F{}, F{});
+                            else run_chunks(N0{}, N0{}, F{}, F{});
                         } else if (!FM) {
-                            if (aligned) run_chunks(N2{}, N2{}, F{});
-                            else if (small) run_chunks(N2{}, N1{}, F{});
-                            else run_chunks(N2{}, N0{}, F{});
+                            if (atab) run_chunks(N2{}, N2{}, F{}, T{});
+                            else if (aligned) run_chunks(N2{}, N2{}, F{}, F{});
+                            else if (small) run_chunks(N2{}, N1{}, F{}, F{});
+                            else run_chunks(N2{}, N0{}, F{}, F{});
                         }
                         c16 += (run - 1u) * kChunk;
                         dbg_t_run += S2R_DBG_NOW() - dbg_tr0;
```

New measurement: 1487 billion. -10.7%, worse.
